# Ben-Bussch/Lunar_Module_Ascent_Trajectory_Optimiser

Hardware: AMD Instinct MI355X
Metric: solved ascent NLPs/sec (N=200 collocation nodes) (higher is better)
Workload: dtype f64; 1 GPU; BASELINE.json configs[2]: 4096-NLP Isp x dry-mass sweep (64x64, Isp 300-320 s, dry mass 2345-2545 kg), N=200 nodes, backward Euler (reference NODES=2), DCOST applied (the script's MV move penalty 1e-05, Launch_Optimiser.py:99, as an l1 term: the model the reference declares); move_penalty=True, batch_per_gpu=4096, global_batch=4096, n_nodes=200, parallelism=problem-sharded x1, gather only, converged=4096, of=4096

## Files before the change

include/ascent.h:

```cpp
#ifndef ASCENT_H
#define ASCENT_H
#include <stdint.h>

#ifdef __cplusplus
extern "C" {
#endif

typedef struct ascent_params {
  double G;
  double M;
  double R0;
  double Ft;
  double M0;
  double mdot;
  double fuel_mass;
  double mass_scalar;
  double ang_acc_max;
  double r_peri;
  double r_apo;
  double T_scale;
  double angle_ub;
  double tf_lb;
  double tf_ub;
  double dcost;
} ascent_params;

typedef struct ascent_opts {
  int32_t n_nodes;
  int32_t scheme;
  int32_t max_iter;
  int32_t warm_start;
  double tol;
  double mu_init;
  int32_t formulation;
  int32_t coarse_nodes;
  int32_t terminal;
  int32_t solver_path;
  int32_t move_penalty;
  int32_t reserved;
} ascent_opts;

enum ascent_status {
  ASCENT_OK = 0,
  ASCENT_E_ARG = -1,
  ASCENT_E_HIP = -2,
  ASCENT_E_NODEVICE = -3,
  ASCENT_E_NOMEM = -4,
  ASCENT_E_NOTERM = -5
};

enum ascent_problem_status {
  ASCENT_CONVERGED = 0,
  ASCENT_MAX_ITER = 1,
  ASCENT_LINESEARCH_FAILED = 2,
  ASCENT_REGULARISATION_FAILED = 3
};

#define ASCENT_BLOB_ROWS(n_nodes) (21 * ((n_nodes) - 1) + 10)
#define ASCENT_TRAJ_FIELDS 10

int ascent_version(void);
int ascent_device_count(void);
const char *ascent_strerror(int code);

int ascent_solve_batch(const ascent_params *p, int64_t batch, const ascent_opts *o,
                       const double *guess_or_null, double *traj_out, double *tf_out,
                       int32_t *status_out, int32_t *iters_out, double *sol_blob_out_or_null,
                       int device_id, void *hip_stream_or_null, int ptr_is_device);

int ascent_eval_nodes(const ascent_params *p, int64_t batch, const ascent_opts *o,
                      const double *iterate, double *defects, double *jac_blocks,
                      double *hess_blocks, int device_id);

int ascent_kkt_step(const ascent_params *p, int64_t batch, const ascent_opts *o,
                    const double *iterate, const double *mu, const double *delta_w, double *step,
                    int32_t *inertia_out, int device_id);

enum ascent_path { ASCENT_PATH_AUTO = 0, ASCENT_PATH_FUSED = 1, ASCENT_PATH_SPLIT_LANE = 2, ASCENT_PATH_SPLIT_WIDE = 3,
                   ASCENT_PATH_DENSE = 4,
                   ASCENT_PATH_PERSIST = 5  };
int ascent_default_path(int64_t batch, const ascent_opts *o);
int ascent_workspace_layout(int64_t batch, const ascent_opts *o, int64_t *out4);
int ascent_eval_nodes_path(const ascent_params *p, int64_t batch, const ascent_opts *o,
                           const double *iterate, double *defects, double *jac_blocks,
                           double *hess_blocks, int device_id, int path);
int ascent_kkt_step_path(const ascent_params *p, int64_t batch, const ascent_opts *o,
                         const double *iterate, const double *mu, const double *delta_w, double *step,
                         int32_t *inertia_out, int device_id, int path);

int ascent_dense_records(const ascent_params *p, int64_t batch, const ascent_opts *o, const double *iterate,
                         double *records, int device_id);

int ascent_coast_batch(const ascent_params *p, int64_t batch, const double *final_state, int32_t coast_nodes,
                       double *coast_traj, double *coast_tf, double *apsides, int device_id,
                       void *hip_stream_or_null, int ptr_is_device);

int ascent_param_sensitivity(const ascent_params *p, int64_t batch, const ascent_opts *o,
                             const double *sol_blob, double *grad_out,
                             int device_id, void *hip_stream_or_null, int ptr_is_device);

#define ASCENT_FLIGHT_ROWS 10
#define ASCENT_FLIGHT_MAX_SUBSTEPS 4096
int ascent_fly_batch(const ascent_params *p, int64_t batch, const ascent_opts *o, const double *sol_blob,
                     int32_t substeps, double *flown_traj_out_or_null, double *local_err_out_or_null,
                     double *summary_out, int device_id, void *hip_stream_or_null, int ptr_is_device);

int ascent_flight_jacobian(const ascent_params *p, int64_t batch, const ascent_opts *o, const double *sol_blob,
                           int32_t substeps, double *jac_out, double *jac_u_out_or_null, int device_id,
                           void *hip_stream_or_null, int ptr_is_device);

#define ASCENT_TRIM_ROWS 10
int ascent_trim_batch(const ascent_params *p, int64_t batch, const ascent_opts *o, const double *sol_blob, int32_t substeps,
                      int32_t rounds, double tol, double *trim_blob_out, double *summary_out, int device_id,
                      void *hip_stream_or_null, int ptr_is_device);

#define ASCENT_DISPERSE_COLS 24
#define ASCENT_DISPERSE_ROWS 9
#define ASCENT_DISPERSE_STAT_ROWS 82
#define ASCENT_DISPERSE_MAX_SAMPLES 65536
int ascent_disperse_batch(const ascent_params *p, int64_t batch, const ascent_opts *o, const double *sol_blob,
                          int32_t substeps, int32_t samples, const double *xi, const double *sigma,
                          const double *sigma_u_or_null, double *stats_out, double *samples_out_or_null, int device_id,
                          void *hip_stream_or_null, int ptr_is_device);

#define ASCENT_GUIDE_ROWS 5
int ascent_guidance_gains(const ascent_params *p, int64_t batch, const ascent_opts *o, const double *sol_blob, int32_t substeps,
                          const double *weights, double *gain_u_out, double *gain_t_out, double *summary_out,
                          double *jac_cl_out_or_null, double *jac_u_cl_out_or_null, int device_id, void *hip_stream_or_null,
                          int ptr_is_device);

#define ASCENT_GUIDED_SAMPLE_ROWS 12
int ascent_disperse_guided_batch(const ascent_params *p, int64_t batch, const ascent_opts *o, const double *sol_blob,
                                 int32_t substeps, int32_t samples, const double *xi, const double *sigma,
                                 const double *sigma_u_or_null, const double *gain_u, const double *gain_t_or_null,
                                 const double *stretch_max_or_null, double *stats_out, double *samples_out_or_null,
                                 int device_id, void *hip_stream_or_null, int ptr_is_device);

#define ASCENT_NAV_ROWS 8
#define ASCENT_GUIDE_FF_ROWS 7
int ascent_guidance_feedforward(const ascent_params *p, int64_t batch, const ascent_opts *o, const double *sol_blob,
                                int32_t substeps, const double *weights, const double *ff_dir, const double *ff_know_or_null,
                                double *gain_u_out, double *gain_t_out, double *ff_u_out, double *ff_t_out, double *summary_out,
                                double *jac_cl_out_or_null, double *jac_u_cl_out_or_null, double *jac_nav_out_or_null,
                                int device_id, void *hip_stream_or_null, int ptr_is_device);

int ascent_disperse_navigated_batch(const ascent_params *p, int64_t batch, const ascent_opts *o, const double *sol_blob,
                                    int32_t substeps, int32_t samples, const double *xi, const double *sigma,
                                    const double *sigma_u_or_null, const double *gain_u, const double *gain_t_or_null,
                                    const double *stretch_max_or_null, const double *ff_u_or_null, const double *ff_t_or_null,
                                    const double *ff_know_or_null, const double *xi_nav_or_null, const double *sigma_nav_or_null,
                                    double *stats_out, double *samples_out_or_null, int device_id, void *hip_stream_or_null,
                                    int ptr_is_device);

#define ASCENT_HISTORY_QUANTITIES 10
#define ASCENT_HISTORY_ROWS 52
int ascent_disperse_history_batch(const ascent_params *p, int64_t batch, const ascent_opts *o, const double *sol_blob,
                                  int32_t substeps, int32_t samples, const double *xi, const double *sigma,
                                  const double *sigma_u_or_null, const double *gain_u_or_null, const double *gain_t_or_null,
                                  const double *stretch_max_or_null, const double *ff_u_or_null, const double *ff_t_or_null,
                                  const double *ff_know_or_null, const double *xi_nav_or_null, const double *sigma_nav_or_null,
                                  int32_t node_stride, double *stats_out, double *samples_out_or_null, double *hist_out,
                                  double *hist_samples_out_or_null, int device_id, void *hip_stream_or_null, int ptr_is_device);

int ascent_kkt_solve(int64_t batch, int32_t n_nodes, int32_t bs, int32_t nb, const double *diag, const double *lower,
                     const double *upper, const double *border, const double *border_diag, const double *rhs,
                     double *sol, int device_id, int algo);

double ascent_last_kernel_ms(int device_id);

#ifdef __cplusplus
}
#endif
#endif
```

lunar_module_ascent_trajectory_optimiser_amd/_lib.py:

```python
from __future__ import annotations

import ctypes as C
import os

HERE = os.path.dirname(os.path.abspath(__file__))
LIB_PATH = os.path.join(HERE, "csrc", "libascent.so")

_dp = C.POINTER(C.c_double)
_ip = C.POINTER(C.c_int32)


class AscentParamsC(C.Structure):
    _fields_ = [(n, C.c_double) for n in (
        "G", "M", "R0", "Ft", "M0", "mdot", "fuel_mass", "mass_scalar", "ang_acc_max", "r_peri",
        "r_apo", "T_scale", "angle_ub", "tf_lb", "tf_ub", "dcost")]


class AscentOptsC(C.Structure):
    _fields_ = [("n_nodes", C.c_int32), ("scheme", C.c_int32), ("max_iter", C.c_int32),
                ("warm_start", C.c_int32), ("tol", C.c_double), ("mu_init", C.c_double),
                ("formulation", C.c_int32), ("coarse_nodes", C.c_int32), ("terminal", C.c_int32),
                ("solver_path", C.c_int32), ("move_penalty", C.c_int32), ("reserved", C.c_int32)]


SYMBOLS = ("ascent_version", "ascent_device_count", "ascent_strerror", "ascent_solve_batch",
           "ascent_eval_nodes", "ascent_kkt_step", "ascent_eval_nodes_path", "ascent_kkt_step_path",
           "ascent_dense_records", "ascent_coast_batch", "ascent_kkt_solve", "ascent_last_kernel_ms", "ascent_default_path",
           "ascent_workspace_layout", "ascent_param_sensitivity", "ascent_fly_batch", "ascent_flight_jacobian",
           "ascent_trim_batch", "ascent_disperse_batch", "ascent_guidance_gains", "ascent_disperse_guided_batch",
           "ascent_guidance_feedforward", "ascent_disperse_navigated_batch", "ascent_disperse_history_batch")
PATHS = {"auto": 0, "fused": 1, "split_lane": 2, "split_wide": 3, "dense": 4, "persist": 5}

_lib = None


class AscentLibraryError(RuntimeError):
    pass


def hip_runtimes_mapped() -> list[str]:
    seen = []
    try:
        with open("/proc/self/maps") as f:
            for line in f:
                path = line.rsplit(None, 1)[-1] if "/" in line else ""
                if "libamdhip64" in os.path.basename(path) and path not in seen:
                    seen.append(path)
    except OSError:
        pass
    return seen


def _bind_hip_runtime():
    if hip_runtimes_mapped() or os.environ.get("ASCENT_HIP_RUNTIME", "auto") == "system":
        return
    import importlib.util
    try:
        spec = importlib.util.find_spec("torch")
    except (ImportError, ValueError):
        spec = None
    if spec is None or not spec.origin:
        return
    cand = os.path.join(os.path.dirname(spec.origin), "lib", "libamdhip64.so")
    if os.path.exists(cand):
        try:
            C.CDLL(cand, mode=C.RTLD_GLOBAL)
        except OSError as e:
            import warnings
            warnings.warn(f"could not map {cand} ({e}); libascent.so binds to the system HIP runtime")


def require_single_hip_runtime():
    m = hip_runtimes_mapped()
    if len(m) > 1:
        raise AscentLibraryError(
            "two HIP runtimes are mapped into this process (" + ", ".join(m) + "): libascent.so was bound to one before torch "
            "loaded the other, so torch's device pointers and streams cannot be handed to it.  Import this package with "
            "ASCENT_HIP_RUNTIME unset (it then maps torch's runtime first), or `import torch` before the first solve.")


def load():
    global _lib
    if _lib is not None:
        return _lib
    if not os.path.exists(LIB_PATH):
        raise AscentLibraryError(
            f"{LIB_PATH} not found: build it with `python -m lunar_module_ascent_trajectory_optimiser_amd.build` "
            "(hipcc --offload-arch=gfx950).  There is no CPU fallback.")
    _bind_hip_runtime()
    L = C.CDLL(LIB_PATH)
    for s in SYMBOLS:
        if not hasattr(L, s):
            raise AscentLibraryError(f"{LIB_PATH} does not export {s}")
    L.ascent_version.restype = C.c_int
    L.ascent_device_count.restype = C.c_int
    L.ascent_strerror.restype = C.c_char_p
    L.ascent_strerror.argtypes = [C.c_int]
    L.ascent_last_kernel_ms.restype = C.c_double
    L.ascent_last_kernel_ms.argtypes = [C.c_int]
    L.ascent_solve_batch.restype = C.c_int
    L.ascent_solve_batch.argtypes = [C.c_void_p, C.c_int64, C.POINTER(AscentOptsC), C.c_void_p, C.c_void_p,
                                     C.c_void_p, C.c_void_p, C.c_void_p, C.c_void_p, C.c_int, C.c_void_p, C.c_int]
    L.ascent_eval_nodes.restype = C.c_int
    L.ascent_eval_nodes.argtypes = [C.c_void_p, C.c_int64, C.POINTER(AscentOptsC), C.c_void_p, C.c_void_p,
                                    C.c_void_p, C.c_void_p, C.c_int]
    L.ascent_kkt_step.restype = C.c_int
    L.ascent_kkt_step.argtypes = [C.c_void_p, C.c_int64, C.POINTER(AscentOptsC), C.c_void_p, C.c_void_p,
                                  C.c_void_p, C.c_void_p, C.c_void_p, C.c_int]
    L.ascent_eval_nodes_path.restype = C.c_int
    L.ascent_eval_nodes_path.argtypes = L.ascent_eval_nodes.argtypes + [C.c_int]
    L.ascent_kkt_step_path.restype = C.c_int
    L.ascent_kkt_step_path.argtypes = L.ascent_kkt_step.argtypes + [C.c_int]
    L.ascent_default_path.restype = C.c_int
    L.ascent_default_path.argtypes = [C.c_int64, C.POINTER(AscentOptsC)]
    L.ascent_workspace_layout.restype = C.c_int
    L.ascent_workspace_layout.argtypes = [C.c_int64, C.POINTER(AscentOptsC), C.POINTER(C.c_int64)]
    L.ascent_dense_records.restype = C.c_int
    L.ascent_dense_records.argtypes = [C.c_void_p, C.c_int64, C.POINTER(AscentOptsC), C.c_void_p, C.c_void_p, C.c_int]
    L.ascent_kkt_solve.restype = C.c_int
    L.ascent_kkt_solve.argtypes = [C.c_int64, C.c_int32, C.c_int32, C.c_int32] + [C.c_void_p] * 7 + [C.c_int, C.c_int]
    L.ascent_coast_batch.restype = C.c_int
    L.ascent_coast_batch.argtypes = [C.c_void_p, C.c_int64, C.c_void_p, C.c_int32, C.c_void_p, C.c_void_p, C.c_void_p,
                                     C.c_int, C.c_void_p, C.c_int]
    L.ascent_param_sensitivity.restype = C.c_int
    L.ascent_param_sensitivity.argtypes = [C.c_void_p, C.c_int64, C.POINTER(AscentOptsC), C.c_void_p, C.c_void_p, C.c_int,
                                           C.c_void_p, C.c_int]
    L.ascent_fly_batch.restype = C.c_int
    L.ascent_fly_batch.argtypes = [C.c_void_p, C.c_int64, C.POINTER(AscentOptsC), C.c_void_p, C.c_int32, C.c_void_p, C.c_void_p,
                                   C.c_void_p, C.c_int, C.c_void_p, C.c_int]
    L.ascent_flight_jacobian.restype = C.c_int
    L.ascent_flight_jacobian.argtypes = [C.c_void_p, C.c_int64, C.POINTER(AscentOptsC), C.c_void_p, C.c_int32, C.c_void_p, C.c_void_p,
                                         C.c_int, C.c_void_p, C.c_int]
    L.ascent_trim_batch.restype = C.c_int
    L.ascent_trim_batch.argtypes = [C.c_void_p, C.c_int64, C.POINTER(AscentOptsC), C.c_void_p, C.c_int32, C.c_int32, C.c_double,
                                    C.c_void_p, C.c_void_p, C.c_int, C.c_void_p, C.c_int]
    L.ascent_disperse_batch.restype = C.c_int
    L.ascent_disperse_batch.argtypes = [C.c_void_p, C.c_int64, C.POINTER(AscentOptsC), C.c_void_p, C.c_int32, C.c_int32, C.c_void_p,
                                        C.c_void_p, C.c_void_p, C.c_void_p, C.c_void_p, C.c_int, C.c_void_p, C.c_int]
    L.ascent_guidance_gains.restype = C.c_int
    L.ascent_guidance_gains.argtypes = [C.c_void_p, C.c_int64, C.POINTER(AscentOptsC), C.c_void_p, C.c_int32] + [C.c_void_p] * 6 + [
        C.c_int, C.c_void_p, C.c_int]
    L.ascent_disperse_guided_batch.restype = C.c_int
    L.ascent_disperse_guided_batch.argtypes = [C.c_void_p, C.c_int64, C.POINTER(AscentOptsC), C.c_void_p, C.c_int32, C.c_int32] + [
        C.c_void_p] * 8 + [C.c_int, C.c_void_p, C.c_int]
    L.ascent_guidance_feedforward.restype = C.c_int
    L.ascent_guidance_feedforward.argtypes = [C.c_void_p, C.c_int64, C.POINTER(AscentOptsC), C.c_void_p, C.c_int32] + [C.c_void_p] * 11 + [
        C.c_int, C.c_void_p, C.c_int]
    L.ascent_disperse_navigated_batch.restype = C.c_int
    L.ascent_disperse_navigated_batch.argtypes = [C.c_void_p, C.c_int64, C.POINTER(AscentOptsC), C.c_void_p, C.c_int32, C.c_int32] + [
        C.c_void_p] * 13 + [C.c_int, C.c_void_p, C.c_int]
    L.ascent_disperse_history_batch.restype = C.c_int
    L.ascent_disperse_history_batch.argtypes = [C.c_void_p, C.c_int64, C.POINTER(AscentOptsC), C.c_void_p, C.c_int32, C.c_int32] + [
        C.c_void_p] * 11 + [C.c_int32] + [C.c_void_p] * 4 + [C.c_int, C.c_void_p, C.c_int]
    _lib = L
    return L


def check(rc: int):
    if rc != 0:
        raise AscentLibraryError(f"libascent error {rc}: {load().ascent_strerror(rc).decode()}")
```

lunar_module_ascent_trajectory_optimiser_amd/csrc/ascent_dense.hip:

```cpp
#include <hip/hip_runtime.h>

#include <cstdio>
#include <cstdlib>

#include "ascent.h"
#include "ascent_device.hpp"
#include "ascent_tile.hpp"
#include "ascent_dense.hpp"
#include "ascent_blocktri.hpp"
#include "ascent_flight_dev.hpp"

using namespace ascent;

namespace {

constexpr int NIT = 26;
constexpr int O_Z = 0, O_U = 7, O_L = 8, O_ZB = 15;
constexpr int O_LU = 21, O_PP = 22, O_PN = 23, O_ZP = 24, O_ZN = 25;
constexpr int NV_GA = 0, NV_GB = 8, NV_P = 16, NNV = 27;
constexpr int G_JA = 0, G_JB = 1, G_HAA = 2, G_HAB = 3, G_HBB = 4, G_V = 5, NGRID = 6;
constexpr int F_EA = 0, F_LA = 1, F_EL2 = 2, F_GAIN = 3;
constexpr int FWD_DOUBLES = 3 * 64 + 16;
enum {
  X_STATE, X_ITERS, X_STATUS, X_CUR, X_FIRST, X_LS, X_MU, X_NUP, X_DWL, X_ALPHA, X_ADU, X_PHI0, X_DM, X_C1, X_SL,
// ... 8 lines not shown
struct DGeo {
  int K, scheme, terminal, dc;
  __host__ __device__ size_t nlp_doubles() const {
    return (size_t)K * (3 * NIT + NNV + NGRID * 64 + FWD_DOUBLES) + NSCAL;
  }
  __host__ __device__ size_t off_it(int buf) const { return (size_t)buf * NIT * K; }
  __host__ __device__ size_t off_st() const { return (size_t)2 * NIT * K; }
  __host__ __device__ size_t off_nv() const { return (size_t)3 * NIT * K; }
  __host__ __device__ size_t off_rec() const { return (size_t)(3 * NIT + NNV) * K; }
  __host__ __device__ size_t off_fwd() const { return off_rec() + (size_t)K * NGRID * 64; }
  __host__ __device__ size_t off_sc() const { return off_fwd() + (size_t)K * FWD_DOUBLES; }
};

ASC_DEV Scal load_scal(const double *sc, int r0) {
  Scal s;
  s.th = sc[r0 + S_TH]; s.zlt = sc[r0 + S_ZLT]; s.zut = sc[r0 + S_ZUT]; s.s1 = sc[r0 + S_S1]; s.s2 = sc[r0 + S_S2];
  s.zs1 = sc[r0 + S_ZS1]; s.zs2 = sc[r0 + S_ZS2]; s.nu3 = sc[r0 + S_NU3]; s.nu1 = sc[r0 + S_NU1]; s.nu2 = sc[r0 + S_NU2];
  return s;
}
ASC_DEV void store_scal(double *sc, int r0, const Scal &s) {
  sc[r0 + S_TH] = s.th; sc[r0 + S_ZLT] = s.zlt; sc[r0 + S_ZUT] = s.zut; sc[r0 + S_S1] = s.s1; sc[r0 + S_S2] = s.s2;
  sc[r0 + S_ZS1] = s.zs1; sc[r0 + S_ZS2] = s.zs2; sc[r0 + S_NU3] = s.nu3; sc[r0 + S_NU1] = s.nu1; sc[r0 + S_NU2] = s.nu2;
}
ASC_DEV Scal trial_scal(const Der &d, const Scal &s, const Scal &ds, double alpha, double adu, double mu, bool first) {
  Scal t = s;
  if (first) return t;
  t.th += alpha * ds.th; t.s1 += alpha * ds.s1; t.s2 += alpha * ds.s2;
  t.nu3 += alpha * ds.nu3; t.nu1 += alpha * ds.nu1; t.nu2 += alpha * ds.nu2;
  t.zlt = clipz(s.zlt + adu * ds.zlt, t.th - d.tlb, mu);
  t.zut = clipz(s.zut + adu * ds.zut, d.tub - t.th, mu);
  t.zs1 = clipz(s.zs1 + adu * ds.zs1, t.s1, mu);
  t.zs2 = clipz(s.zs2 + adu * ds.zs2, t.s2, mu);
  return t;
}

__global__ __launch_bounds__(WAVE) void d_init(const ascent_params *params, long batch, DGeo g, double *ws,
                                               const double *guess, int warm, double mu_init, int probe,
                                               const double *probe_mu) {
  const long p = blockIdx.y;
  const int k = blockIdx.x * WAVE + threadIdx.x, K = g.K;
  if (k >= K) return;
  double *w = ws + (size_t)p * g.nlp_doubles();
  const Der d = derive_t(params[p], g.terminal);
  const int asked_warm = warm;
  if (warm && !(guess[(21L * K + S_TH) * batch + p] > 0.0)) warm = 0;
  const double tf0 = 0.9, dr = 0.166, aend = 0.5, vp = sqrt(d.vp2), dt0 = (1.0 / K) * d.T * tf0;
  const double sdr = sin(dr), cdr = cos(dr);
  const double xf = -d.rhof * sdr, yf = d.rhof * cdr - d.rho0;
  double z[7], l[7], zb[6], u;
  if (warm) {
    ASC_UNROLL
    for (int i = 0; i < 7; i++) {
      z[i] = guess[(7L * k + i) * batch + p];
      l[i] = guess[(8L * K + 7L * k + i) * batch + p];
    }
    u = guess[(7L * K + k) * batch + p];
    ASC_UNROLL
    for (int b = 0; b < 6; b++) zb[b] = guess[(15L * K + 6L * k + b) * batch + p];
  } else {
    const double fr = (double)(k + 1) / K;
    z[IX] = fr * xf; z[IY] = fr * yf; z[IVX] = -fr * vp * cdr; z[IVY] = -fr * vp * sdr; z[IA] = fr * aend;
    z[IW] = aend / (K * dt0); z[IM] = d.mrate * dt0 * (k + 1);
    u = 0.0;
  }
  if (!probe) {
    z[IA] = push_in(z[IA], 0.0, d.aub);
    z[IM] = push_in(z[IM], 0.0, 1.0);
    u = push_in(u, -1.0, 1.0);
  }
  ASC_UNROLL
  for (int b = 0; b < 6; b++) zb[b] = warm == 2 ? (probe ? zb[b] : fmax(zb[b], 1e-12)) : 1.0;
  ASC_UNROLL
  for (int i = 0; i < 7; i++) l[i] = warm == 2 ? l[i] : 0.0;
  double *it = w + g.off_it(0), *st = w + g.off_st();
  ASC_UNROLL
  for (int i = 0; i < 7; i++) { it[(O_Z + i) * K + k] = z[i]; it[(O_L + i) * K + k] = l[i]; }
  it[O_U * K + k] = u;
  ASC_UNROLL
  for (int b = 0; b < 6; b++) it[(O_ZB + b) * K + k] = zb[b];
  for (int r = 0; r < NIT; r++) st[r * K + k] = 0.0;
  if (g.dc) {
    double up = (k > 0 && warm) ? guess[(7L * K + k - 1) * batch + p] : 0.0;
    if (k > 0 && !probe) up = push_in(up, -1.0, 1.0);
    const double dl = u - up, eps = warm ? 1e-4 : 1e-2, dc = params[p].dcost;
    it[O_LU * K + k] = 0.0;
    it[O_PP * K + k] = fmax(dl, 0.0) + eps; it[O_PN * K + k] = fmax(-dl, 0.0) + eps;
    it[O_ZP * K + k] = dc; it[O_ZN * K + k] = dc;
  }
  if (k != K - 1) return;
  double *sc = w + g.off_sc();
  Scal s;
  if (warm) {
    const double *gs = guess + (21L * K) * batch + p;
    s.th = gs[S_TH * batch]; s.zlt = gs[S_ZLT * batch]; s.zut = gs[S_ZUT * batch]; s.s1 = gs[S_S1 * batch];
    s.s2 = gs[S_S2 * batch]; s.zs1 = gs[S_ZS1 * batch]; s.zs2 = gs[S_ZS2 * batch]; s.nu3 = gs[S_NU3 * batch];
    s.nu1 = gs[S_NU1 * batch]; s.nu2 = gs[S_NU2 * batch];
  } else {
    s.th = tf0;
  }
  if (!probe) s.th = push_in(s.th, d.tlb, d.tub);
  const Terminal tm = terminal_of(d, z);
  if (probe) {
  } else if (warm != 2) {
    s.s1 = fmax(tm.g1, 1e-2); s.s2 = fmax(tm.g2, 1e-2);
    s.zlt = s.zut = s.zs1 = s.zs2 = 1.0;
    s.nu3 = s.nu1 = s.nu2 = 0.0;
  } else {
    s.s1 = fmax(s.s1, 1e-10); s.s2 = fmax(s.s2, 1e-10);
    s.zlt = fmax(s.zlt, 1e-12); s.zut = fmax(s.zut, 1e-12);
    s.zs1 = fmax(s.zs1, 1e-12); s.zs2 = fmax(s.zs2, 1e-12);
  }
  for (int r = 0; r < NSCAL; r++) sc[r] = 0.0;
  store_scal(sc, X_S, s);
  sc[X_STATE] = ST_TRIAL; sc[X_FIRST] = 1.0; sc[X_STATUS] = ASCENT_MAX_ITER;
  sc[X_MU] = probe ? probe_mu[p] : ((asked_warm && !warm) ? 0.1 : mu_init);
  sc[X_NUP] = 1.0;
}

struct QMap { int q; double c; };

ASC_DEV void h4_full(const double *H10, double H4[4][4]) {
  H4[0][0] = H10[0]; H4[0][1] = H4[1][0] = H10[1]; H4[0][2] = H4[2][0] = H10[2]; H4[0][3] = H4[3][0] = H10[3];
  H4[1][1] = H10[4]; H4[1][2] = H4[2][1] = H10[5]; H4[1][3] = H4[3][1] = H10[6];
  H4[2][2] = H10[7]; H4[2][3] = H4[3][2] = H10[8]; H4[3][3] = H10[9];
}

__global__ __launch_bounds__(WAVE) void d_eval(const ascent_params *params, long batch, DGeo g, double *ws) {
  const long p = blockIdx.y;
  const int k = blockIdx.x * WAVE + threadIdx.x, K = g.K;
  double *w = ws + (size_t)p * g.nlp_doubles();
  double *sc = w + g.off_sc();
  if ((int)sc[X_STATE] != ST_TRIAL || k >= K) return;
  const Der d = derive_t(params[p], g.terminal);
  const bool first = sc[X_FIRST] != 0.0;
  const double alpha = first ? 0.0 : sc[X_ALPHA], adu = first ? 0.0 : sc[X_ADU], mu = sc[X_MU];
  const Scal s = load_scal(sc, X_S), ds = load_scal(sc, X_D);
  const Scal stt = trial_scal(d, s, ds, alpha, adu, mu, first);
  const int cur = (int)sc[X_CUR];
  const double *ic = w + g.off_it(cur), *st = w + g.off_st();
  double *in = w + g.off_it(1 - cur), *nv = w + g.off_nv(), *rec = w + g.off_rec() + (size_t)k * NGRID * 64;
  const double hT = (1.0 / K) * d.T, dt = hT * stt.th;
  const double wa = g.scheme == 0 ? 0.0 : g.scheme == 1 ? 0.5 : 1.0 / 6.0;
  const double wm = g.scheme == 2 ? 4.0 / 6.0 : 0.0;
  const double wb = g.scheme == 0 ? 1.0 : g.scheme == 1 ? 0.5 : 1.0 / 6.0;
  const double sa = dt * wa, sm = dt * wm, sb = dt * wb, e8 = 0.125 * dt, h8 = 0.125 * hT;
  double za[7], zb[7], lam[7], zbd[6], u;
  ASC_UNROLL
  for (int i = 0; i < 7; i++) {
    zb[i] = ic[(O_Z + i) * K + k] + alpha * st[(O_Z + i) * K + k];
    za[i] = k ? ic[(O_Z + i) * K + k - 1] + alpha * st[(O_Z + i) * K + k - 1] : 0.0;
    lam[i] = ic[(O_L + i) * K + k] + alpha * st[(O_L + i) * K + k];
  }
  u = ic[O_U * K + k] + alpha * st[O_U * K + k];
  const double dist[6] = {zb[IA], d.aub - zb[IA], zb[IM], 1.0 - zb[IM], u + 1.0, 1.0 - u};
  const double mlo = mu * 1e-10, mhi = mu * 1e10;
  ASC_UNROLL
  for (int b = 0; b < 6; b++) {
    double v = ic[(O_ZB + b) * K + k];
    if (!first) { const double id = rcp(dist[b]); v = fmin(fmax(v + adu * st[(O_ZB + b) * K + k], mlo * id), mhi * id); }
    zbd[b] = v;
    in[(O_ZB + b) * K + k] = v;
  }
  ASC_UNROLL
  for (int i = 0; i < 7; i++) { in[(O_Z + i) * K + k] = zb[i]; in[(O_L + i) * K + k] = lam[i]; }
  in[O_U * K + k] = u;
  double lu = 0.0, pp = 1.0, pn = 1.0, zp = 0.0, zn = 0.0, cu = 0.0;
  if (g.dc) {
    const double up = k ? ic[O_U * K + k - 1] + alpha * st[O_U * K + k - 1] : 0.0;
    lu = ic[O_LU * K + k] + alpha * st[O_LU * K + k];
    pp = ic[O_PP * K + k] + alpha * st[O_PP * K + k];
    pn = ic[O_PN * K + k] + alpha * st[O_PN * K + k];
    zp = ic[O_ZP * K + k]; zn = ic[O_ZN * K + k];
    if (!first) {
      const double ip = rcp(pp), in_ = rcp(pn);
      zp = fmin(fmax(zp + adu * st[O_ZP * K + k], mlo * ip), mhi * ip);
      zn = fmin(fmax(zn + adu * st[O_ZN * K + k], mlo * in_), mhi * in_);
    }
    in[O_LU * K + k] = lu; in[O_PP * K + k] = pp; in[O_PN * K + k] = pn; in[O_ZP * K + k] = zp; in[O_ZN * K + k] = zn;
    cu = u - up - pp + pn;
  }
  if (k == K - 1) store_scal(sc, X_T, stt);
  double Ga[8], Gb[8], Gm[8], Hw[10], fa[7], fb[7], fm[7], zm[7], ax, ay;
  ASC_UNROLL
  for (int i = 0; i < 8; i++) { Ga[i] = 0.0; Gm[i] = 0.0; }
  ASC_UNROLL
  for (int i = 0; i < 7; i++) { fa[i] = 0.0; fm[i] = 0.0; zm[i] = 0.0; }
  accel<1>(d, zb[IX], zb[IY], zb[IA], zb[IM], 0.0, 0.0, ax, ay, Gb, nullptr);
  rhs_f(d, zb, u, ax, ay, fb);
  if (g.scheme != 0) {
    accel<1>(d, za[IX], za[IY], za[IA], za[IM], 0.0, 0.0, ax, ay, Ga, nullptr);
    rhs_f(d, za, u, ax, ay, fa);
  }
  double H4m[4][4];
  ASC_UNROLL
  for (int i = 0; i < 4; i++) {
    ASC_UNROLL
    for (int j = 0; j < 4; j++) H4m[i][j] = 0.0;
  }
  double gm[7], mth[7];
// ... 1170 lines not shown
```

lunar_module_ascent_trajectory_optimiser_amd/csrc/ascent_hs.hip:

```cpp
#include <hip/hip_runtime.h>

#pragma clang fp contract(on)

#include <cstdio>
#include <cstdlib>

#include "ascent.h"
#include "ascent_device.hpp"
#include "ascent_tile.hpp"
#include "ascent_persist.hpp"
#include "ascent_persist_dev.hpp"

using namespace ascent;

namespace {

typedef __attribute__((address_space(3))) double ldbl;
constexpr int HCH = 12, HCW = 48;
constexpr int LDH = 49;
constexpr int H_GA = 0, H_GM = 8, H_GB = 16, H_EB = 24, H_ES = 28, H_W = 32, H_R0 = 42, H_C = 45, H_JT = 52, H_H = 59, H_RZ = 69,
              H_GT = 76, H_ROWS = 83;
constexpr int C_PSI = 0, C_GA = 7, C_HA = 14, C_WA = 21, C_OM = 23, C_TG = 27, C_N = 34;


// ... 306 lines not shown
    ASC_UNROLL
    for (int i = 0; i < 10; i++) stage[(H_W + i) * LDH + col] = -sm * pt.Hm[i];
    ASC_UNROLL
    for (int i = 0; i < 7; i++) { stage[(H_C + i) * LDH + col] = cc[i]; stage[(H_JT + i) * LDH + col] = Jth[i]; }
  }
  double gan[7], han[7], wan[2];
  ASC_UNROLL
  for (int i = 0; i < 7; i++) { gan[i] = __shfl_down(q.ga[i], 1); han[i] = __shfl_down(Hath[i], 1); }
  wan[0] = __shfl_down(q.wa[0], 1); wan[1] = __shfl_down(q.wa[1], 1);
  if (on) {
    if (k == K - 1) {
      ASC_UNROLL
      for (int i = 0; i < 7; i++) { gan[i] = 0.0; han[i] = 0.0; }
      wan[0] = 0.0; wan[1] = 0.0;
    } else if (lastl) {
      ASC_UNROLL
      for (int i = 0; i < 7; i++) { gan[i] = carry[C_GA + i]; han[i] = carry[C_HA + i]; }
      wan[0] = carry[C_WA]; wan[1] = carry[C_WA + 1];
    }
    double Hn[10], Gx[8], t1, t2;
    accel<2>(d, z[IX], z[IY], z[IA], z[IM], q.wb[0] + wan[0], q.wb[1] + wan[1], t1, t2, Gx, Hn);
    const double dist[6] = {z[IA], d.aub - z[IA], z[IM], 1.0 - z[IM], u + 1.0, 1.0 - u};
    double id[6];
    ASC_UNROLL
    for (int b = 0; b < 6; b++) id[b] = rcp(dist[b]);
    ASC_UNROLL
    for (int i = 0; i < 10; i++) Hn[i] = -Hn[i];
    Hn[7] += zb6[0] * id[0] + zb6[1] * id[1];
    Hn[9] += zb6[2] * id[2] + zb6[3] * id[3];
    ASC_UNROLL
    for (int i = 0; i < 10; i++) stage[(H_H + i) * LDH + col] = Hn[i];
    ASC_UNROLL
    for (int i = 0; i < 7; i++) {
      double rz = q.gb[i] + gan[i];
      if (i == IA) rz += mu * (id[1] - id[0]);
      if (i == IM) rz += mu * (id[3] - id[2]);
      stage[(H_RZ + i) * LDH + col] = rz;
      stage[(H_GT + i) * LDH + col] = Hbth[i] + han[i];
    }
    stage[H_R0 * LDH + col] = zb6[4] * id[4] + zb6[5] * id[5] + dw;
    stage[(H_R0 + 1) * LDH + col] = -bu * lw + mu * (id[5] - id[4]);
    stage[(H_R0 + 2) * LDH + col] = -hT * d.alpha * lw;
  }
  wsync();
  if (on && firstl) {
    ASC_UNROLL
    for (int i = 0; i < 7; i++) { carry[C_GA + i] = q.ga[i]; carry[C_HA + i] = Hath[i]; }
    carry[C_WA] = q.wa[0]; carry[C_WA + 1] = q.wa[1];
  }
  wsync();
  return Hthth;
}

constexpr int F_OUT = 49, A_RHS = 42, A_C = 49, A_J = 56;
template <int WIDE>
ASC_PASS double hs_eval_forward(const ldbl *dp, const gdbl *it, const gdbl *gains, ldbl *stage, int K, int Kp, int kn, bool on, int nl, int col,
                                double h, double hT, double dth, double dnu3, double carry_m) {
  const Der d = der_load(dp);
  const double bu = h * d.alpha;
  double x0m = 0.0, du00 = 0.0, ka[7], rc[7];
  HsJ J;
  if (on) {
    double z[7], zp[7];
    ASC_UNROLL
    for (int i = 0; i < 7; i++) {
      z[i] = it[(O_Z + i) * Kp + kn];
      const double pv = it[(O_Z + i) * Kp + (kn > 0 ? kn - 1 : 0)];
      zp[i] = kn > 0 ? pv : 0.0;
    }
    const double u_ = it[O_U * Kp + kn];
    ASC_UNROLL
    for (int i = 0; i < 7; i++) ka[i] = gains[(size_t)i * Kp + kn];
    du00 = -(gains[(size_t)7 * Kp + kn] + gains[(size_t)8 * Kp + kn] * dth + gains[(size_t)9 * Kp + kn] * dnu3);
    HsPts pt;
    hs_points<0>(d, zp, z, u_, h, 0.0, 0.0, pt);
    double cc[7], Jth[7], eb[4], es[4];
    hs_defect(pt, zp, z, h, hT, cc, Jth);
    hs_blocks(pt.Gb, pt.Gm, h, eb, es);
    hs_coeffs(pt.Ga, pt.Gm, pt.Gb, eb, es, h, bu, J);
    ASC_UNROLL
    for (int i = 0; i < 7; i++) rc[i] = cc[i] + Jth[i] * dth;
    x0m = -rc[IM];
  }
  double incl = x0m;
  ASC_UNROLL
  for (int sft = 1; sft < (WIDE ? 64 : 16); sft *= 2) {
    const double t = __shfl_up(incl, sft, WIDE ? 64 : 16);
    if (nl >= sft) incl += t;
  }
  const double dzm_k = carry_m + incl, dzm_p = dzm_k - x0m;
  carry_m += WIDE ? __shfl(incl, HCW - 1) : bcast16<HCH - 1>(incl);
  if (on) {
    constexpr int NC = 6, FS = 7;
    const double du00p = du00 - ka[IM] * dzm_p;
    double X[4][7], Ab[4][7];
    hs_rows(J, X, Ab);
    auto emit = [&](int i, const double *xr_, const double *ar) {
      const double bw = bu * xr_[IW];
      double v = bw * du00p + ar[IM] * dzm_p;
      ASC_UNROLL
      for (int j = 0; j < 7; j++) v -= xr_[j] * rc[j];
      ASC_UNROLL
      for (int j = 0; j < 6; j++) stage[(FS * i + j) * LDH + col] = ar[j] - bw * ka[j];
      stage[(FS * i + NC) * LDH + col] = v;
    };
    emit(IX, X[0], Ab[0]); emit(IY, X[1], Ab[1]); emit(IVX, X[2], Ab[2]); emit(IVY, X[3], Ab[3]);
    {
      const double xa[7] = {0, 0, 0, 0, 1.0, 0.5 * h, 0}, aa[7] = {0, 0, 0, 0, 1.0, h, 0};
      emit(IA, xa, aa);
      const double xw[7] = {0, 0, 0, 0, 0, 1.0, 0}, aw[7] = {0, 0, 0, 0, 0, 1.0, 0};
      emit(IW, xw, aw);
    }
    ASC_UNROLL
    for (int j = 0; j < 6; j++) stage[(42 + j) * LDH + col] = -ka[j];
    stage[48 * LDH + col] = du00p;
    stage[(F_OUT + 6) * LDH + col] = dzm_k;
  }
  wsync();
  return carry_m;
}

template <int TERM>
ASC_PASS double hs_eval_adjoint(const ldbl *dp, const ldbl *sc, const gdbl *it, const gdbl *stp, ldbl *stage, ldbl *carry, int K, int Kp, int kn,
                                bool on, bool lastl, bool firstl, int col, double h, double hT, double mu, double dw, double dth, double dnu3) {
  const Der d = der_load(dp);
  const double bu = h * d.alpha, e8 = 0.125 * h;
  double ccl = 0.0, ccn[7], rhs[7] = {0, 0, 0, 0, 0, 0, 0};
  double om[4] = {0, 0, 0, 0}, Hath[7] = {0, 0, 0, 0, 0, 0, 0}, Hbth[7];
  HsJ J;
  HsPts pt;
  HsDual q;
  ASC_UNROLL
  for (int i = 0; i < 7; i++) q.ga[i] = 0.0;
  q.wa[0] = 0.0; q.wa[1] = 0.0;
  double z[7], dz[7], zb6[4];
  if (on) {
    double zp[7], l[7], dzp[7];
    ASC_UNROLL
    for (int i = 0; i < 7; i++) {
      const int km = kn > 0 ? kn - 1 : 0;
      z[i] = it[(O_Z + i) * Kp + kn]; l[i] = it[(O_L + i) * Kp + kn]; dz[i] = stp[(O_Z + i) * Kp + kn];
      const double pv = it[(O_Z + i) * Kp + km], dpv = stp[(O_Z + i) * Kp + km];
      zp[i] = kn > 0 ? pv : 0.0; dzp[i] = kn > 0 ? dpv : 0.0;
    }
    const double u = it[O_U * Kp + kn];
    ASC_UNROLL
    for (int b = 0; b < 4; b++) zb6[b] = it[(O_ZB + b) * Kp + kn];
    hs_points<1>(d, zp, z, u, h, l[IVX], l[IVY], pt);
    hs_dual(pt, l, h, q);
    double Jth[7], Hthth, eb[4], es[4];
    hs_defect(pt, zp, z, h, hT, ccn, Jth);
    hs_theta(pt, q, h, hT, Hath, Hbth, Hthth);
    hs_blocks(pt.Gb, pt.Gm, h, eb, es);
    hs_coeffs(pt.Ga, pt.Gm, pt.Gb, eb, es, h, bu, J);
    ASC_UNROLL
    for (int i = 0; i < 7; i++) ccl += ccn[i] * l[i];
    const double xi[4] = {0.5 * (dzp[IX] + dz[IX]) + e8 * (dzp[IVX] - dz[IVX]), 0.5 * (dzp[IY] + dz[IY]) + e8 * (dzp[IVY] - dz[IVY]),
                          0.5 * (dzp[IA] + dz[IA]) + e8 * (dzp[IW] - dz[IW]), 0.5 * (dzp[IM] + dz[IM])};
    const double sm = (4.0 / 6.0) * h;
    const double *H = pt.Hm;
    om[0] = -sm * (H[0] * xi[0] + H[1] * xi[1] + H[2] * xi[2] + H[3] * xi[3]);
    om[1] = -sm * (H[1] * xi[0] + H[4] * xi[1] + H[5] * xi[2] + H[6] * xi[3]);
    om[2] = -sm * (H[2] * xi[0] + H[5] * xi[1] + H[7] * xi[2] + H[8] * xi[3]);
    om[3] = -sm * (H[3] * xi[0] + H[6] * xi[1] + H[8] * xi[2] + H[9] * xi[3]);
  }
  double gan[7], han[7], wan[2], omn[4];
  ASC_UNROLL
  for (int i = 0; i < 7; i++) { gan[i] = __shfl_down(q.ga[i], 1); han[i] = __shfl_down(Hath[i], 1); }
  wan[0] = __shfl_down(q.wa[0], 1); wan[1] = __shfl_down(q.wa[1], 1);
  ASC_UNROLL
  for (int r = 0; r < 4; r++) omn[r] = __shfl_down(om[r], 1);
  if (on) {
// ... 693 lines not shown
```

lunar_module_ascent_trajectory_optimiser_amd/csrc/ascent_persist.hip:

```cpp
#include <hip/hip_runtime.h>

#pragma clang fp contract(on)

#include <cstdio>
#include <cstdlib>

#include "ascent.h"
#include "ascent_device.hpp"
#include "ascent_tile.hpp"
#include "ascent_persist.hpp"
#include "ascent_persist_dev.hpp"

using namespace ascent;

namespace {


ASC_DEV void start_move(double *w, int Kp, int k, double u, double up, bool warm, double dcw) {
  const double dl = u - up, eps = warm ? 1e-4 : 1e-2;
  w[(R_IT + O_LU) * Kp + k] = 0.0;
  w[(R_IT + O_PP) * Kp + k] = fmax(dl, 0.0) + eps;
  w[(R_IT + O_PN) * Kp + k] = fmax(-dl, 0.0) + eps;
  w[(R_IT + O_ZP) * Kp + k] = dcw;
  w[(R_IT + O_ZN) * Kp + k] = dcw;
}
struct MovePivot { double ip, in_, sgp, sgn, rp, rn, Rd, gdl; };
ASC_DEV MovePivot move_pivot(double pp, double pn, double zp, double zn, double lu, double dcw, double mu, double dw) {
  MovePivot m;
  m.ip = rcp(pp); m.in_ = rcp(pn);
  m.sgp = zp * m.ip + dw; m.sgn = zn * m.in_ + dw;
  m.rp = dcw - mu * m.ip - lu; m.rn = dcw - mu * m.in_ + lu;
  const double isp = rcp(m.sgp), isn = rcp(m.sgn);
  m.Rd = rcp(isp + isn);
  m.gdl = m.Rd * (m.rp * isp - m.rn * isn);
  return m;
}

ASC_DEV void start_node(const Der &d, int K, int kk, int warm, bool probe, int form, double *z, double *l, double *zb, double &u) {
  if (!warm) {
    const double tf0 = 0.9, dr = 0.166, aend = 0.5, vp = sqrt(d.vp2), dt0 = (1.0 / K) * d.T * tf0;
    const double sdr = sin(dr), cdr = cos(dr);
    const double xf = -d.rhof * sdr, yf = d.rhof * cdr - d.rho0;
    const double fr = (double)(kk + 1) / K;
    z[IX] = fr * xf; z[IY] = fr * yf; z[IVX] = -fr * vp * cdr; z[IVY] = -fr * vp * sdr; z[IA] = fr * aend;
    z[IW] = aend / (K * dt0); z[IM] = d.mrate * dt0 * (kk + 1);
    u = 0.0;
    if (form == 1) {
      z[IW] = 0.0;
      u = z[IA] / (0.5 * d.aub) - 1.0;
    }
  }
  if (!probe) {
    z[IA] = push_in(z[IA], 0.0, d.aub);
    z[IM] = push_in(z[IM], 0.0, 1.0);
    u = push_in(u, -1.0, 1.0);
  }
  ASC_UNROLL
  for (int b = 0; b < 6; b++) zb[b] = probe ? zb[b] : warm == 2 ? fmax(zb[b], 1e-12) : 1.0;
  ASC_UNROLL
  for (int i = 0; i < 7; i++) l[i] = warm == 2 ? l[i] : 0.0;
}
ASC_DEV void start_scal(const Der &d, int warm, bool probe, const double *zK, Scal &s) {
  if (!warm) s.th = 0.9;
  if (!probe) s.th = push_in(s.th, d.tlb, d.tub);
  const Terminal tm = terminal_of(d, zK);
  if (probe) {
  } else if (warm != 2) {
    s.s1 = fmax(tm.g1, 1e-2); s.s2 = fmax(tm.g2, 1e-2);
    s.zlt = s.zut = s.zs1 = s.zs2 = 1.0;
    s.nu3 = s.nu1 = s.nu2 = 0.0;
  } else {
    s.s1 = fmax(s.s1, 1e-10); s.s2 = fmax(s.s2, 1e-10);
    s.zlt = fmax(s.zlt, 1e-12); s.zut = fmax(s.zut, 1e-12);
    s.zs1 = fmax(s.zs1, 1e-12); s.zs2 = fmax(s.zs2, 1e-12);
  }
}
ASC_DEV void store_start(double *w, int Kp, int k, const double *z, const double *l, const double *zb, double u) {
  ASC_UNROLL
  for (int i = 0; i < 7; i++) { w[(R_IT + O_Z + i) * Kp + k] = z[i]; w[(R_IT + O_L + i) * Kp + k] = l[i]; }
  w[(R_IT + O_U) * Kp + k] = u;
  ASC_UNROLL
  for (int b = 0; b < 6; b++) w[(R_IT + O_ZB + b) * Kp + k] = zb[b];
}

__global__ __launch_bounds__(WAVE) void p_init(const ascent_params *params, long batch, PGeo g, double *ws, const double *guess,
                                               int warm, double mu_init, const double *probe_mu, const double *probe_dw, int probe_kind) {
  const long p = blockIdx.y;
  const int k = blockIdx.x * WAVE + threadIdx.x, K = g.K, Kp = g.Kp;
  if (k >= Kp) return;
  double *w = ws + (size_t)p * g.nlp_doubles();
  const Der d = derive_t(params[p], g.term);
  const int asked_warm = warm;
  if (warm && !(guess[(21L * K + S_TH) * batch + p] > 0.0)) warm = 0;
  const bool probe = probe_mu != nullptr;
  double z[7], l[7], zb[6], u = 0.0;
  const int kk = k < K ? k : K - 1;
  if (warm) {
    ASC_UNROLL
    for (int i = 0; i < 7; i++) { z[i] = guess[(7L * kk + i) * batch + p]; l[i] = guess[(8L * K + 7L * kk + i) * batch + p]; }
    u = guess[(7L * K + kk) * batch + p];
    ASC_UNROLL
    for (int b = 0; b < 6; b++) zb[b] = guess[(15L * K + 6L * kk + b) * batch + p];
  }
  start_node(d, K, kk, warm, probe, g.form, z, l, zb, u);
  store_start(w, Kp, k, z, l, zb, u);
  if (g.mp) {
    const double ha = 0.5 * d.aub, f0 = (double)kk / K * 0.5;
    double up = kk == 0 ? (g.form == 1 ? -1.0 : 0.0) : warm ? guess[(7L * K + kk - 1) * batch + p] : (g.form == 1 ? f0 / ha - 1.0 : 0.0);
    if (kk > 0 && !probe) up = push_in(up, -1.0, 1.0);
    start_move(w, Kp, k, u, up, warm != 0, g.form == 1 ? params[p].dcost * ha : params[p].dcost);
  }
  if (k != K - 1) return;
  double *sc = w + (size_t)g.nrows() * Kp;
  Scal s;
  if (warm) {
    const double *gs = guess + (21L * K) * batch + p;
    s.th = gs[S_TH * batch]; s.zlt = gs[S_ZLT * batch]; s.zut = gs[S_ZUT * batch]; s.s1 = gs[S_S1 * batch];
    s.s2 = gs[S_S2 * batch]; s.zs1 = gs[S_ZS1 * batch]; s.zs2 = gs[S_ZS2 * batch]; s.nu3 = gs[S_NU3 * batch];
    s.nu1 = gs[S_NU1 * batch]; s.nu2 = gs[S_NU2 * batch];
  }
  start_scal(d, warm, probe, z, s);
  for (int r = 0; r < NSCAL; r++) sc[r] = 0.0;
  put_scal(sc, X_S, s);
  sc[X_STATE] = ST_TRIAL; sc[X_FIRST] = 1.0; sc[X_STATUS] = ASCENT_MAX_ITER;
  sc[X_MU] = (asked_warm && !warm) ? 0.1 : mu_init; sc[X_NUP] = 1.0;
  if (probe) { sc[X_MU] = probe_mu[p]; sc[X_PDW] = probe_dw[p]; sc[X_PROBE] = (double)probe_kind; }
}

__global__ __launch_bounds__(WAVE) void p_transfer(const ascent_params *params, long batch, PGeo gc, const double *wsc, PGeo gf,
                                                   double *wsf, double mu) {
  const long p = blockIdx.y;
  const int k = blockIdx.x * WAVE + threadIdx.x, Kc = gc.K, Kf = gf.K, Kpc = gc.Kp, Kpf = gf.Kp;
  if (k >= Kpf) return;
  const double *wc = wsc + (size_t)p * gc.nlp_doubles(), *scc = wc + (size_t)gc.nrows() * Kpc;
  double *wf = wsf + (size_t)p * gf.nlp_doubles();
  const Der d = derive_t(params[p], gf.term);
  const int warm = (int)scc[X_STATUS] == ASCENT_CONVERGED ? 2 : 0;
  const double *ic = wc + (size_t)((int)scc[X_CUR] * gc.nit()) * Kpc;
  double z[7], l[7], zb[6], u = 0.0, up = 0.0;
  const int kk = k < Kf ? k : Kf - 1;
  if (warm && gf.mp && kk > 0) {
    const double x = (double)kk / (double)Kf * (double)Kc;
    int j = (int)x;
    if (j > Kc - 1) j = Kc - 1;
    const double wt = x - (double)j;
    const int ja = j ? j - 1 : 0;
    const double a = ic[O_U * Kpc + ja], b = ic[O_U * Kpc + j];
    up = push_in(fma(wt, b - a, a), -1.0, 1.0);
  }
  if (warm) {
    const double x = (double)(kk + 1) / (double)Kf * (double)Kc;
    int j = (int)x;
    if (j > Kc - 1) j = Kc - 1;
    const double wt = x - (double)j;
    const int ja = j ? j - 1 : 0;
    const double zsc = (double)Kc / (double)Kf;
    ASC_UNROLL
    for (int i = 0; i < 7; i++) {
      const double a = j ? ic[(O_Z + i) * Kpc + ja] : ((gf.form == 1 && i == IA) ? ic[(O_Z + i) * Kpc] : 0.0), b = ic[(O_Z + i) * Kpc + j];
      z[i] = fma(wt, b - a, a);
      const double la = ic[(O_L + i) * Kpc + ja], lb = ic[(O_L + i) * Kpc + j];
      l[i] = fma(wt, lb - la, la);
    }
    { const double a = ic[O_U * Kpc + ja], b = ic[O_U * Kpc + j]; u = fma(wt, b - a, a); }
    ASC_UNROLL
    for (int b6 = 0; b6 < 6; b6++) {
      const double a = ic[(O_ZB + b6) * Kpc + ja], b = ic[(O_ZB + b6) * Kpc + j];
      zb[b6] = fma(wt, b - a, a) * zsc;
    }
  }
  start_node(d, Kf, kk, warm, false, gf.form, z, l, zb, u);
  store_start(wf, Kpf, k, z, l, zb, u);
  if (gf.mp) {
    if (kk == 0) up = gf.form == 1 ? -1.0 : 0.0;
    else if (!warm && gf.form == 1) up = push_in((double)kk / Kf * 0.5 / (0.5 * d.aub) - 1.0, -1.0, 1.0);
    start_move(wf, Kpf, k, u, up, warm != 0, gf.form == 1 ? params[p].dcost * 0.5 * d.aub : params[p].dcost);
  }
  if (k != Kf - 1) return;
  double *sc = wf + (size_t)gf.nrows() * Kpf;
  Scal s;
  if (warm) s = lds_scal(scc, X_S);
  start_scal(d, warm, false, z, s);
  for (int r = 0; r < NSCAL; r++) sc[r] = 0.0;
  put_scal(sc, X_S, s);
  sc[X_STATE] = ST_TRIAL; sc[X_FIRST] = 1.0; sc[X_STATUS] = ASCENT_MAX_ITER;
  sc[X_MU] = warm ? mu : 0.1; sc[X_NUP] = 1.0;
  sc[X_ITB] = scc[X_ITB] + scc[X_ITERS];
}

constexpr int FIN_WAVES = 8, FIN_SUB = CH / FIN_WAVES;
__global__ __launch_bounds__(WAVE * FIN_WAVES) void p_finish(const ascent_params *params, long batch, PGeo g, const double *ws, double *traj,
                                                 double *tf_out, int *status_out, int *iters_out, double *blob) {
  const long p = (long)blockIdx.y * WAVE + threadIdx.x;
  if (p >= batch) return;
  const int c = blockIdx.x, K = g.K, Kp = g.Kp, nt = K + 1;
  const double *w = ws + (size_t)p * g.nlp_doubles();
  const double *sc = w + (size_t)g.nrows() * Kp;
  const Der d = derive_t(params[p], g.term);
  const double *it = w + (size_t)((int)sc[X_CUR] * g.nit()) * Kp;
  if (c == 0 && threadIdx.y == 0) {
    const Scal s = lds_scal(sc, X_S);
    tf_out[p] = s.th;
    status_out[p] = (int)sc[X_STATUS];
    iters_out[p] = (int)sc[X_ITERS] + (int)sc[X_ITB];
    if (blob) {
      double *bs = blob + (21L * K) * batch + p;
      bs[S_TH * batch] = s.th; bs[S_ZLT * batch] = s.zlt; bs[S_ZUT * batch] = s.zut; bs[S_S1 * batch] = s.s1;
      bs[S_S2 * batch] = s.s2; bs[S_ZS1 * batch] = s.zs1; bs[S_ZS2 * batch] = s.zs2; bs[S_NU3 * batch] = s.nu3;
      bs[S_NU1 * batch] = s.nu1; bs[S_NU2 * batch] = s.nu2;
    }
    if (traj) {
      double ax, ay;
      accel<0>(d, 0.0, 0.0, 0.0, 0.0, 0.0, 0.0, ax, ay, nullptr, nullptr);
      const double v[10] = {0.0, 0.0, 0.0, 0.0, ax, ay, 0.0, 0.0, 0.0, 0.0};
      ASC_UNROLL
      for (int f = 0; f < 10; f++) traj[((long)f * nt) * batch + p] = v[f];
    }
  }
  for (int k = c * CH + threadIdx.y * FIN_SUB; k < min(K, c * CH + (threadIdx.y + 1) * FIN_SUB); k++) {
    double z[7];
    ASC_UNROLL
    for (int q = 0; q < 7; q++) z[q] = it[(O_Z + q) * Kp + k];
    const double u = it[O_U * Kp + k];
    if (blob) {
      ASC_UNROLL
      for (int q = 0; q < 7; q++) {
        blob[(7L * k + q) * batch + p] = z[q];
        blob[(8L * K + 7L * k + q) * batch + p] = it[(O_L + q) * Kp + k];
      }
      blob[(7L * K + k) * batch + p] = u;
      ASC_UNROLL
      for (int b = 0; b < 6; b++) blob[(15L * K + 6L * k + b) * batch + p] = it[(O_ZB + b) * Kp + k];
    }
    if (traj) {
      double ax, ay;
      accel<0>(d, z[IX], z[IY], z[IA], z[IM], 0.0, 0.0, ax, ay, nullptr, nullptr);
      const double v[10] = {z[IX], z[IY], z[IVX], z[IVY], ax, ay, z[IA], z[IW], u, z[IM]};
      ASC_UNROLL
      for (int f = 0; f < 10; f++) traj[((long)f * nt + k + 1) * batch + p] = v[f];
    }
  }
}

__global__ __launch_bounds__(WAVE) void p_probe_out(long batch, PGeo g, const double *ws, double *step, int *inertia) {
  const long p = blockIdx.y;
  const int k = blockIdx.x * WAVE + threadIdx.x, K = g.K, Kp = g.Kp;
  if (k >= K) return;
  const double *w = ws + (size_t)p * g.nlp_doubles();
  const double *sc = w + (size_t)g.nrows() * Kp, *stp = w + (size_t)g.r_st() * Kp;
  const bool ok = (int)sc[X_STATE] == ST_TRIAL;
  if (k == 0) {
    inertia[p] = ok ? 0 : 1;
    for (int r = 0; r < 10; r++) step[(21L * K + r) * batch + p] = ok ? sc[X_D + r] : 0.0;
  }
  ASC_UNROLL
  for (int i = 0; i < 7; i++) {
    step[(7L * k + i) * batch + p] = ok ? stp[(O_Z + i) * Kp + k] : 0.0;
    step[(8L * K + 7L * k + i) * batch + p] = ok ? stp[(O_L + i) * Kp + k] : 0.0;
  }
  step[(7L * K + k) * batch + p] = ok ? stp[O_U * Kp + k] : 0.0;
  ASC_UNROLL
  for (int b = 0; b < 6; b++) step[(15L * K + 6L * k + b) * batch + p] = ok ? stp[(O_ZB + b) * Kp + k] : 0.0;
}

__global__ __launch_bounds__(WAVE) void p_probe_rows_out(const ascent_params *params, long batch, PGeo g, const double *ws, double *defects,
                                                         double *jac, double *hess) {
  const long p = blockIdx.y;
  const int k = blockIdx.x * WAVE + threadIdx.x, K = g.K, Kp = g.Kp;
  if (k >= K) return;
  const double *w = ws + (size_t)p * g.nlp_doubles();
  const double *sc = w + (size_t)g.nrows() * Kp, *rows = w + (size_t)g.r_st() * Kp;
  const double *it = w + (size_t)((int)sc[X_CUR] * g.nit()) * Kp;
  const Der d = derive_t(params[p], g.term);
  const double a_ = it[(O_Z + IA) * Kp + k], m_ = it[(O_Z + IM) * Kp + k];
  const double siga = it[(O_ZB + 0) * Kp + k] * rcp(a_) + it[(O_ZB + 1) * Kp + k] * rcp(d.aub - a_);
  const double sigm = it[(O_ZB + 2) * Kp + k] * rcp(m_) + it[(O_ZB + 3) * Kp + k] * rcp(1.0 - m_);
  ASC_UNROLL
  for (int i = 0; i < 8; i++) jac[(8L * k + i) * batch + p] = rows[i * Kp + k];
  ASC_UNROLL
  for (int i = 0; i < 10; i++) hess[(10L * k + i) * batch + p] = rows[(8 + i) * Kp + k] - (i == 7 ? siga : i == 9 ? sigm : 0.0);
  ASC_UNROLL
  for (int i = 0; i < 7; i++) defects[(7L * k + i) * batch + p] = rows[(18 + i) * Kp + k];
}


template <int FORM>
ASC_DEV void ainv_vrows(const double *G, const double *E, double dt, double *rvx, double *rvy) {
  double c1[7], c2[7];
  c1[IX] = dt * G[0]; c1[IY] = dt * G[1]; c1[IVX] = 1.0; c1[IVY] = 0.0; c1[IA] = dt * G[2]; c1[IW] = FORM == 1 ? 0.0 : dt * c1[IA]; c1[IM] = dt * G[3];
  c2[IX] = dt * G[4]; c2[IY] = dt * G[5]; c2[IVX] = 0.0; c2[IVY] = 1.0; c2[IA] = dt * G[6]; c2[IW] = FORM == 1 ? 0.0 : dt * c2[IA]; c2[IM] = dt * G[7];
  ASC_UNROLL
  for (int i = 0; i < 7; i++) { rvx[i] = E[0] * c1[i] + E[1] * c2[i]; rvy[i] = E[2] * c1[i] + E[3] * c2[i]; }
}


struct TrialKeep { double G[8], F[7], dza, dzm, zb4, zb5, zpp, zpn; };

template <int SCHEME, int FORM, int MP = 0, int TERM = 0>
ASC_DEV void trial_primal(const Der &d, int K, int Kp, int k, const NodeIn &n, const NodeIn &dn, const TrialCtx &t, bool live,
                          double *in, Part &P, TrialKeep &kp) {
  const double alpha = t.alpha;
  double z[7], zp[7], zb[6];
  ASC_UNROLL
  for (int i = 0; i < 7; i++) { z[i] = n.z[i] + alpha * dn.z[i]; zp[i] = n.zp[i] + alpha * dn.zp[i]; }
  const double u = n.u + alpha * dn.u;
  const double dist[6] = {z[IA], d.aub - z[IA], z[IM], 1.0 - z[IM], u + 1.0, 1.0 - u};
  ASC_UNROLL
  for (int b = 0; b < 6; b++) {
    const double id = rcp(dist[b]);
    zb[b] = t.first ? n.zb[b] : fmin(fmax(n.zb[b] + t.adu * dn.zb[b], t.mlo * id), t.mhi * id);
  }
  if (live) {
    ASC_UNROLL
    for (int i = 0; i < 7; i++) in[(O_Z + i) * Kp + k] = z[i];
    in[O_U * Kp + k] = u;
    ASC_UNROLL
    for (int b = 0; b < 6; b++) in[(O_ZB + b) * Kp + k] = zb[b];
  }
  kp.zpp = 0.0; kp.zpn = 0.0;
  if constexpr (MP) {
    const double up = n.up + alpha * dn.up, pp = n.pp + alpha * dn.pp, pn = n.pn + alpha * dn.pn;
    const double ip = rcp(pp), in_ = rcp(pn);
    const double zpp = t.first ? n.zpp : fmin(fmax(n.zpp + t.adu * dn.zpp, t.mlo * ip), t.mhi * ip);
    const double zpn = t.first ? n.zpn : fmin(fmax(n.zpn + t.adu * dn.zpn, t.mlo * in_), t.mhi * in_);
// ... 97 lines not shown
                        double *in, Part &P) {
  TrialKeep kp;
  trial_primal<SCHEME, FORM, MP, TERM>(d, K, Kp, k, n, dn, t, live, in, P, kp);
  double l[7], ln[7];
  ASC_UNROLL
  for (int i = 0; i < 7; i++) { l[i] = n.l[i] + t.alpha * dn.l[i]; ln[i] = n.ln[i] + t.alpha * dn.ln[i]; }
  const double lu = MP ? n.lu + t.alpha * dn.lu : 0.0, lun = MP ? n.lun + t.alpha * dn.lun : 0.0;
  trial_dual<SCHEME, FORM, MP, TERM>(d, K, Kp, k, kp, l, ln, lu, lun, t, live, in, P);
}


template <int SCHEME, int FORM, int MP = 0, int TERM = 0, int WIDE = 0>
__global__ __launch_bounds__(WAVE) void p_solve(const ascent_params *params, long batch, PGeo g, double *ws, int max_iter, double tol) {
  using L = Lay<MP>;
  constexpr int NS = L::NS, NIT = L::NIT, R_ST = L::R_ST, R_KA = L::R_KA, R_K0 = L::R_K0, NROWS = L::NROWS;
  constexpr int S_G = L::S_G, S_E = L::S_E, S_H = L::S_H, S_F = L::S_F, S_C = L::S_C, S_RZ = L::S_RZ, S_GT = L::S_GT, S_SC = L::S_SC;
  constexpr int RL = NS;
  static_assert(FORM == 0 || SCHEME == 0, "the v1 formulation is restated with backward Euler");
  __shared__ double stage[L::S_ROWS * LDW];
  __shared__ double outb[L::OUT_ROWS * LDW];
  __shared__ double lds_t[NPW][NS][NS];
  __shared__ double lds_d[NPW][3][8];
  __shared__ double lsc[NPW][NSCAL];
  __shared__ double lds_c[NPW][8];
  constexpr int CHN = WIDE ? 64 : CH;
  const int lane = threadIdx.x, grp = lane >> 4, role = lane & 15;
  const int nl = WIDE ? lane : role;
  const int cbase = WIDE ? 0 : grp * 16;
  const long p = WIDE ? (long)blockIdx.x : (long)blockIdx.x * NPW + grp;
  const bool live = p < batch;
  const long pc = live ? p : batch - 1;
  const int K = g.K, Kp = g.Kp, nch = g.nch;
  double *w = ws + (size_t)pc * g.nlp_doubles();
  double *gsc = w + (size_t)NROWS * Kp;
  double *sc = lsc[WIDE ? 0 : grp];
  const Der d = TERM == 2 ? derive_t(params[pc], 2) : derive(params[pc]);
  static_assert(TERM == 0 || (TERM == 2 && FORM == 0), "terminal 2 is carried for the current formulation");
  for (int r = role; r < NSCAL; r += 16) sc[r] = gsc[r];
  if (role < 8) lds_d[grp][2][role] = 0.0;
  wsync();
  if (!live && role == 0) sc[X_STATE] = ST_DONE;
  wsync();
  const int col = grp * 16 + role;
  const double hT = (1.0 / K) * d.T;
  constexpr int IB = FORM == 1 ? IA : IW;
  const double dcw = MP ? (FORM == 1 ? params[pc].dcost * 0.5 * d.aub : params[pc].dcost) : 0.0;
  constexpr double UINIT = FORM == 1 ? -1.0 : 0.0;

  PROF_DECL
  for (int round = 0; round < 64 * (max_iter + 2); round++) {
    PROF(9);
    int state = (int)sc[X_STATE];
    if (__all(state == ST_DONE)) break;
    int pass = 0;
    do {
      if (state == ST_TRIAL) {
        const bool first = sc[X_FIRST] != 0.0;
        const double alpha = first ? 0.0 : sc[X_ALPHA], adu = first ? 0.0 : sc[X_ADU], mu = sc[X_MU];
        const Scal s = lds_scal(sc, X_S), ds = lds_scal(sc, X_D);
        const Scal stt = trial_scal(d, s, ds, alpha, adu, mu, first);
        const int cur = (int)sc[X_CUR];
        const double *ic = w + (size_t)(cur * NIT) * Kp, *stp = w + (size_t)R_ST * Kp;
        double *in = w + (size_t)((1 - cur) * NIT) * Kp;
        const double dt = hT * stt.th, be = dt * d.alpha;
        const double mlo = mu * 1e-10, mhi = mu * 1e10;
        Part P;
        if (sc[X_TEVAL] != 0.0) {
          P.rd = sc[X_P + 0]; P.cinf = sc[X_P + 1]; P.pmin = sc[X_P + 2]; P.pmax = sc[X_P + 3]; P.l1 = sc[X_P + 4];
          P.zsum = sc[X_P + 5]; P.rth = sc[X_P + 6]; P.c1 = sc[X_P + 7]; P.sl = sc[X_P + 8]; P.mv = sc[X_P + 9];
        } else {
          TrialCtx t;
          t.alpha = alpha; t.adu = adu; t.mlo = mlo; t.mhi = mhi; t.dt = dt; t.be = be; t.hT = hT; t.first = first; t.stt = stt; t.dcw = dcw;
          P.clear();
          for (int c = 0; c < nch; c++) {
            const int k = c * CHN + nl;
            if (k < K) {
              NodeIn n, dn;
              load_node<MP>(ic, Kp, K, k, n, UINIT);
              if (first) dn = NodeIn{};
              else load_node<MP>(stp, Kp, K, k, dn);
              trial_node<SCHEME, FORM, MP, TERM>(d, K, Kp, k, n, dn, t, live, in, P);
            }
          }
          P.template reduceW<MP, WIDE>();
        }
        double rd = P.rd, cinf = P.cinf, pmin = P.pmin, pmax = P.pmax, l1 = P.l1, zsum = P.zsum;
        const double rth = 1.0 + P.rth, c1 = P.c1, sl = P.sl;
        double nu_pen = sc[X_NUP], iters = sc[X_ITERS], mu2 = mu;
        int nstate = ST_FACTOR;
        bool accepted = true;
        if (!first) {
          const double phi0 = sc[X_PHI0], Dm = sc[X_DM];
          const double phit = (MP ? stt.th + dcw * P.mv : stt.th) - mu * sl + nu_pen * c1;
          if (!(isfinite(phit) && phit <= phi0 + 1e-8 * alpha * Dm + 2.220446049250313e-15 * fabs(phi0))) {
            accepted = false;
            const int ls = (int)sc[X_LS] + 1;
            wsync();
            if (role == 0) {
              sc[X_LS] = ls; sc[X_TEVAL] = 0.0;
              if (ls >= 40) { sc[X_STATUS] = ASCENT_LINESEARCH_FAILED; sc[X_STATE] = ST_DONE; }
              else sc[X_ALPHA] = 0.5 * alpha;
            }
          } else {
            iters += 1.0;
          }
        }
        if (accepted) {
          ErrParts e;
          e.rd = fmax(rd, fabs(rth - stt.zlt + stt.zut));
          e.rd = fmax(e.rd, fmax(fabs(-stt.nu1 - stt.zs1), fabs(-stt.nu2 - stt.zs2)));
          e.cinf = cinf;
          const double pr[4] = {(stt.th - d.tlb) * stt.zlt, (d.tub - stt.th) * stt.zut, stt.s1 * stt.zs1, stt.s2 * stt.zs2};
          ASC_UNROLL
          for (int q = 0; q < 4; q++) { pmin = fmin(pmin, pr[q]); pmax = fmax(pmax, pr[q]); }
          e.pmin = pmin; e.pmax = pmax;
          l1 += fabs(stt.nu3) + fabs(stt.nu1) + fabs(stt.nu2);
          zsum += stt.zlt + stt.zut + stt.zs1 + stt.zs2;
          e.sd = fmax(100.0, (l1 + zsum) / (double)((MP ? 16 : 13) * K + 7)) * 0.01;
          int status = -1;
          const bool probe = sc[X_PROBE] != 0.0;
          if (probe) { }
          else if (e.err(0.0) <= tol) { status = ASCENT_CONVERGED; nstate = ST_DONE; }
          else if ((int)iters >= max_iter) { status = ASCENT_MAX_ITER; nstate = ST_DONE; }
          else {
            while (mu2 > tol * 0.1 && e.err(mu2) <= 10.0 * mu2) {
              mu2 = fmax(tol * 0.1, fmin(0.2 * mu2, mu2 * sqrt(mu2)));
              nu_pen = 1.0;
            }
          }
#ifdef PERSIST_TRACE
          if (role == 0 && p == PERSIST_TRACE && K > 100)
            printf("[persist] K=%d iter %2d mu %.1e E0 %.2e (dual %.1e primal %.1e compl %.1e..%.1e s_d %.2g) alpha %.3g adu %.3g ls %d dw %.1e nu_pen %.2g c1 %.2e\n", K, (int)iters, mu,
                   e.err(0.0), e.rd, e.cinf, e.pmin, e.pmax, e.sd, alpha, adu, (int)sc[X_LS], sc[X_DWL], nu_pen, c1);
          if (role == 0 && p == PERSIST_TRACE && K > 100)
            printf("[persist]      dual rows: nodes %.2e | th %.2e s1 %.2e s2 %.2e\n", rd, fabs(rth - stt.zlt + stt.zut), fabs(-stt.nu1 - stt.zs1), fabs(-stt.nu2 - stt.zs2));
#endif
          wsync();
          if (role == 0) {
            put_scal(sc, X_S, stt);
            sc[X_CUR] = 1 - cur; sc[X_FIRST] = 0.0; sc[X_ITERS] = iters; sc[X_LS] = 0.0; sc[X_C1] = c1; sc[X_SL] = sl; sc[X_RTH] = rth;
            sc[X_MU] = mu2; sc[X_NUP] = nu_pen; sc[X_DW] = probe ? sc[X_PDW] : 0.0; sc[X_STATE] = nstate; sc[X_TEVAL] = 0.0;
            if (MP) sc[X_MV] = P.mv;
            if (status >= 0) sc[X_STATUS] = status;
          }
        }
      }
      wsync();
      state = (int)sc[X_STATE];
    } while (__builtin_expect(__any(state == ST_TRIAL) && ++pass < 41, 0));
    PROF(0);
    state = (int)sc[X_STATE];
    if (__any(state == ST_FACTOR)) {
      const bool act = state == ST_FACTOR;
      const Scal s = lds_scal(sc, X_S);
      const double mu = sc[X_MU], dw = sc[X_DW];
      const double *it = w + (size_t)((int)sc[X_CUR] * NIT) * Kp;
      const double dt = hT * s.th, be = dt * d.alpha, ith = rcp(s.th), cs = SCHEME == 1 ? 0.5 * dt : dt;
      const double ha = 0.5 * d.aub, bu = FORM == 1 ? ha : be;
      const double hTc = SCHEME == 1 ? 0.5 * hT : hT;
      int grow[NS];
      double gsgn[NS];
      {
        constexpr int hmap[8] = {0, 1, -1, -1, 2, -1, 3, -1};
        constexpr int hrow[4][4] = {{0, 1, 2, 3}, {1, 4, 5, 6}, {2, 5, 7, 8}, {3, 6, 8, 9}};
        ASC_UNROLL
        for (int i = 0; i < NS; i++) {
          int row = S_H; double sgn = 0.0;
// ... 178 lines not shown
              for (int i = 0; i < NS; i++) a[i] += role == i ? dw : 0.0;
            }
            double b[NS];
            solveAT<FORM>(G, E, cs, a, b);
            if constexpr (MP) b[7] = a[7] + bu * b[IB];
            if (colr) {
              ASC_UNROLL
              for (int i = 0; i < NS; i++) lds_t[grp][role][i] = b[i];
              wsync();
              double t[NS];
              ASC_UNROLL
              for (int l2 = 0; l2 < NS; l2++) t[l2] = lds_t[grp][l2][role];
              solveAT<FORM>(G, E, cs, t, b);
              if constexpr (MP) b[7] = t[7] + bu * b[IB];
            }
            double mw[NS], D, coef;
            if constexpr (MP) {
              ASC_UNROLL
              for (int i = 0; i < NS; i++) mw[i] = bcast16<7>(b[i]);
              D = R0 + mw[7];
            } else {
              ASC_UNROLL
              for (int i = 0; i < NS; i++) mw[i] = bu * bcast16<IB>(b[i]);
              D = R0 + dw + bu * mw[IB];
            }
            const double iD = rcp(D);
            if constexpr (MP) {
              const double rsel = role == RL ? ru0 : 0.0;
              coef = (b[7] - rsel) * iD;
            } else {
              const double ru = ru0 + mu * bur, gu = FORM == 1 ? 0.0 : ru0 * ith;
              const double rsel = role == 7 ? ru : role == 8 ? gu : 0.0;
              coef = (bu * b[IB] - rsel) * iD;
            }
            ASC_UNROLL
            for (int i = 0; i < NS; i++) a[i] = b[i] - mw[i] * coef;
            outb[rowK + cj] = role < NS + 3 ? coef : D;
            if (colr) {
              double d0 = 0.0, d1 = 0.0;
              ASC_UNROLL
              for (int i = 0; i < NS; i++) {
                d0 -= a[i] * cc[i];
                if (i < 7) d1 += a[i] * rc1[i];
              }
              lds_d[grp][0][role] = d0;
              lds_d[grp][1][role] = d1;
            }
            wsync();
            {
              double prc[NS];
              ASC_UNROLL
              for (int i = 0; i < NS; i++) prc[i] = lds_d[grp][drow][i];
              double uu = 0.0, vv = 0.0;
              ASC_UNROLL
              for (int i = 0; i < NS; i++) {
                const double pj = a[i] - prc[i], sj = a[i] + pj;
                if (i < 7) uu += rc1[i] * sj;
                vv += cc[i] * sj;
                a[i] = pj;
              }
              U += uu; V += vv;
            }
          }
        }
        wsync();
        PROF(2);
        {
          const int k = c * CHN + nl;
          if (k < K && act) {
            if (live) {
              ASC_UNROLL
              for (int i = 0; i < NS + 3; i++) w[(size_t)(R_KA + i) * Kp + k] = outb[i * LDW + col];
            }
            const double k00 = outb[NS * LDW + col], k01 = outb[(NS + 1) * LDW + col], k02 = outb[(NS + 2) * LDW + col], D = outb[(NS + 3) * LDW + col];
            const double Dk1 = D * k01, Dk2 = D * k02;
            k10 += Dk1 * k00; k11 += Dk1 * k01; k12 += Dk1 * k02; k20 += Dk2 * k00; k22 += Dk2 * k02;
            if (!(D > 0.0)) bad = 1;
          }
        }
        wsync();
        PROF(3);
      }
      const double U0 = bcast16<RL>(U), U1 = bcast16<RL + 1>(U), V1 = bcast16<RL + 1>(V), U2 = bcast16<RL + 2>(U), V2 = bcast16<RL + 2>(V);
      k10 = gsumW<WIDE>(k10); k11 = gsumW<WIDE>(k11); k12 = gsumW<WIDE>(k12); k20 = gsumW<WIDE>(k20); k22 = gsumW<WIDE>(k22);
      bad = (int)gmaxW<WIDE>((double)bad);
      if (probe_rows) {
        if (act && role == 0) sc[X_STATE] = ST_DONE;
      } else if (act) {
        const double S10 = k10 + 0.5 * (U0 - V1), S11 = k11 + U1, S12 = k12 + 0.5 * U2, S20 = k20 - 0.5 * V2, S22 = k22;
        int ok = !bad;
        double dth = 0.0, dnu3 = 0.0;
        if (ok) {
          const double itl = rcp(s.th - d.tlb), itu = rcp(d.tub - s.th);
          const double rthp = sc[X_RTH] + mu * (itu - itl);
          const double sth = s.zlt * itl + s.zut * itu + dw;
          const double a11 = sth - S11, a12 = -S12, a22 = TERM == 2 ? -1.0 : -S22;
          const double b1 = -rthp + S10, b2 = -tm.e3 + S20;
          const double det = a11 * a22 - a12 * a12;
          if (det < 0.0) {
            const double idet = 1.0 / det;
            dth = (b1 * a22 - a12 * b2) * idet;
            dnu3 = (a11 * b2 - a12 * b1) * idet;
          } else {
            ok = 0;
          }
        }
        if (role == 0) {
          if (ok) {
            sc[X_DTH] = dth; sc[X_DNU3] = dnu3; sc[X_SIG1] = sig1; sc[X_SIG2] = sig2; sc[X_RS1] = rs1; sc[X_RS2] = rs2;
            sc[X_CG1] = tm.g1 - s.s1; sc[X_CG2] = tm.g2 - s.s2;
            sc[X_DWL] = dw; sc[X_STATE] = ST_FACTORED;
          } else {
            const double ndw = next_delta_w(dw, sc[X_DWL]);
            if (sc[X_PROBE] != 0.0) sc[X_STATE] = ST_DONE;
            else if (ndw > 1e10) { sc[X_STATUS] = ASCENT_REGULARISATION_FAILED; sc[X_STATE] = ST_DONE; }
            else sc[X_DW] = ndw;
          }
        }
      }
    }
    wsync();
    state = (int)sc[X_STATE];
    if (__any(state == ST_FACTORED)) {
      const bool act = state == ST_FACTORED;
      const Scal s = lds_scal(sc, X_S);
      const double mu = sc[X_MU], dw = sc[X_DWL], dth = sc[X_DTH], dnu3 = sc[X_DNU3];
      const double sig1 = sc[X_SIG1], sig2 = sc[X_SIG2], rs1 = sc[X_RS1], rs2 = sc[X_RS2];
      const double *it = w + (size_t)((int)sc[X_CUR] * NIT) * Kp;
      double *stp = w + (size_t)R_ST * Kp;
      const double dt = hT * s.th, be = dt * d.alpha, cs = SCHEME == 1 ? 0.5 * dt : dt, hTc = SCHEME == 1 ? 0.5 * hT : hT;
      const double ha = 0.5 * d.aub, bu = FORM == 1 ? ha : be;
      const double tau = fmax(0.99, 1.0 - mu);
      {
        constexpr int NC = 6 + MP, FS = NC + 1;
        const int fbase = (role < 7 ? FS * role : 0) * LDW;
        const int fout = (role < 6 ? role : role == 6 ? 7 : 8) * LDW;
        double yown = 0.0, carry_m = 0.0, carry_u = 0.0;
        double rmax = 0.0, gsum = 0.0, adu = 1.0, gmove = 0.0, clu = 0.0;
        double dzK[7] = {0, 0, 0, 0, 0, 0, 0};
        for (int c = 0; c < nch; c++) {
          const int kn = c * CHN + nl;
          const bool on = kn < K && act;
          double a_ = 0.5, m_ = 0.5, u_ = 0.0, zb[6] = {1, 1, 1, 1, 1, 1};
          double G[8], Gp[8], E[4], x0[7], ka[NS], du00 = 0.0;
          double x0u = 0.0, pp_ = 1.0, pn_ = 1.0, zpp_ = 0.0, zpn_ = 0.0, lu_ = 0.0;
          ASC_UNROLL
          for (int i = 0; i < 7; i++) x0[i] = 0.0;
          ASC_UNROLL
          for (int i = 0; i < NS; i++) ka[i] = 0.0;
          if (on) {
            double z[7], zp[7], F[7], ax, ay;
            ASC_UNROLL
            for (int i = 0; i < 7; i++) { z[i] = it[(O_Z + i) * Kp + kn]; zp[i] = kn > 0 ? it[(O_Z + i) * Kp + kn - 1] : 0.0; }
            u_ = it[O_U * Kp + kn];
            a_ = z[IA]; m_ = z[IM];
            ASC_UNROLL
            for (int b = 0; b < 6; b++) zb[b] = it[(O_ZB + b) * Kp + kn];
            ASC_UNROLL
            for (int i = 0; i < NS; i++) ka[i] = w[(size_t)(R_KA + i) * Kp + kn];
            if constexpr (MP) {
              pp_ = it[O_PP * Kp + kn]; pn_ = it[O_PN * Kp + kn]; zpp_ = it[O_ZP * Kp + kn]; zpn_ = it[O_ZN * Kp + kn]; lu_ = it[O_LU * Kp + kn];
              x0u = -(u_ - (kn > 0 ? it[O_U * Kp + kn - 1] : UINIT) - pp_ + pn_);
            }
            du00 = w[(size_t)R_K0 * Kp + kn] + w[(size_t)(R_K0 + 1) * Kp + kn] * dth + w[(size_t)(R_K0 + 2) * Kp + kn] * dnu3;
            accel<1>(d, z[IX], z[IY], z[IA], z[IM], 0.0, 0.0, ax, ay, G, nullptr);
            rhs_f<FORM>(d, z, u_, ax, ay, F);
            if (SCHEME == 1) {
              double Fb[7], axp, ayp;
              accel<1>(d, zp[IX], zp[IY], zp[IA], zp[IM], 0.0, 0.0, axp, ayp, Gp, nullptr);
              rhs_f<FORM>(d, zp, u_, axp, ayp, Fb);
              ASC_UNROLL
              for (int i = 0; i < 7; i++) F[i] = 0.5 * (F[i] + Fb[i]);
            }
            implicit_block(G, cs, E);
            ASC_UNROLL
            for (int i = 0; i < 7; i++) {
              x0[i] = hT * F[i] * dth - ((FORM == 1 && i == IA) ? z[IA] - ha * (u_ + 1.0) : z[i] - zp[i] - dt * F[i]);
              du00 -= ka[i] * x0[i];
            }
            if constexpr (MP) du00 -= ka[7] * x0u;
          }
          double incl = x0[IM];
          ASC_UNROLL
          for (int sft = 1; sft < CHN; sft *= 2) {
            const double t = __shfl_up(incl, sft, CHN);
            if (nl >= sft) incl += t;
          }
          const double dzm_k = carry_m + incl, dzm_p = dzm_k - x0[IM];
          carry_m += WIDE ? __shfl(incl, 63) : bcast16<15>(incl);
          if (on) {
            const double du00p = du00 - ka[IM] * dzm_p;
            double rvx[7], rvy[7];
            ainv_vrows<FORM>(G, E, cs, rvx, rvy);
            auto emit = [&](int i, const double *r, double aw) {
              const double bw = bu * aw;
              if constexpr (MP) stage[(FS * i + 6) * LDW + col] = bw * (1.0 - ka[7]);
              if (SCHEME == 1) {
                double m7[7], t[7];
                ASC_UNROLL
                for (int j = 0; j < 7; j++) m7[j] = r[j] - bw * ka[j];
                fzt_lambda(Gp, m7, t);
                ASC_UNROLL
                for (int j = 0; j < 7; j++) m7[j] += cs * t[j];
                double v = bw * (MP ? x0u + du00 : du00) + m7[IM] * dzm_p;
                ASC_UNROLL
                for (int j = 0; j < 7; j++) v += r[j] * x0[j];
                ASC_UNROLL
                for (int j = 0; j < 6; j++) stage[(FS * i + j) * LDW + col] = m7[j];
                stage[(FS * i + NC) * LDW + col] = v;
                return;
              }
              double v = bw * (MP ? x0u + du00p : du00p) + r[IM] * dzm_p;
              ASC_UNROLL
              for (int j = 0; j < 7; j++) v += r[j] * x0[j];
              ASC_UNROLL
              for (int j = 0; j < 6; j++) stage[(FS * i + j) * LDW + col] = (FORM == 1 && j == IA) ? 0.0 : r[j] - bw * ka[j];
              stage[(FS * i + NC) * LDW + col] = v;
            };
            emit(IVX, rvx, rvx[IB]);
            emit(IVY, rvy, rvy[IB]);
            {
              double r[7];
              ASC_UNROLL
              for (int j = 0; j < 7; j++) r[j] = (j == IX ? 1.0 : 0.0) + cs * rvx[j];
              emit(IX, r, cs * rvx[IB]);
              ASC_UNROLL
              for (int j = 0; j < 7; j++) r[j] = (j == IY ? 1.0 : 0.0) + cs * rvy[j];
              emit(IY, r, cs * rvy[IB]);
              ASC_UNROLL
              for (int j = 0; j < 7; j++) r[j] = j == IA ? 1.0 : (j == IW && FORM == 0) ? cs : 0.0;
              emit(IA, r, FORM == 1 ? 1.0 : cs);
              ASC_UNROLL
              for (int j = 0; j < 7; j++) r[j] = j == IW ? 1.0 : 0.0;
              emit(IW, r, FORM == 1 ? 0.0 : 1.0);
            }
            if constexpr (MP) {
              double kj[7], v0;
              if (SCHEME == 1) {
                double t[7];
                fzt_lambda(Gp, ka, t);
                ASC_UNROLL
                for (int j = 0; j < 7; j++) kj[j] = ka[j] + cs * t[j];
                v0 = du00 - kj[IM] * dzm_p;
              } else {
                ASC_UNROLL
                for (int j = 0; j < 7; j++) kj[j] = ka[j];
                v0 = du00p;
              }
              ASC_UNROLL
              for (int j = 0; j < 6; j++) stage[(FS * 6 + j) * LDW + col] = (FORM == 1 && j == IA) ? 0.0 : -kj[j];
              stage[(FS * 6 + 6) * LDW + col] = 1.0 - ka[7];
              stage[(FS * 6 + NC) * LDW + col] = x0u + v0;
            } else if (SCHEME == 1) {
              double t[7];
              fzt_lambda(Gp, ka, t);
              ASC_UNROLL
              for (int j = 0; j < 6; j++) stage[(42 + j) * LDW + col] = -(ka[j] + cs * t[j]);
              stage[48 * LDW + col] = du00 - (ka[IM] + cs * t[IM]) * dzm_p;
            } else {
              ASC_UNROLL
              for (int j = 0; j < 6; j++) stage[(42 + j) * LDW + col] = (FORM == 1 && j == IA) ? 0.0 : -ka[j];
              stage[48 * LDW + col] = du00p;
            }
            outb[6 * LDW + col] = dzm_k;
          }
          wsync();
          PROF(4);
          if (act) {
            const int jn = min(CHN, K - c * CHN);
            for (int jj = 0; jj < jn; jj++) {
              const int cj = cbase + jj;
              const double *sj = stage + fbase + cj;
              const double m0 = sj[0], m1 = sj[LDW], m2 = sj[2 * LDW], m3 = sj[3 * LDW], m4 = sj[4 * LDW], m5 = sj[5 * LDW], vv = sj[NC * LDW];
              const double b0 = bcast16<0>(yown), b1 = bcast16<1>(yown), b2 = bcast16<2>(yown), b3 = bcast16<3>(yown),
                           b4 = bcast16<4>(yown), b5 = bcast16<5>(yown);
              const double e0 = (vv + m0 * b0) + m2 * b2, e1 = m1 * b1 + m3 * b3, e2 = m4 * b4 + m5 * b5;
              if constexpr (MP) {
                const double m6 = sj[6 * LDW], b6 = bcast16<6>(yown);
                yown = ((e0 + e1) + e2) + m6 * b6;
              } else {
                yown = (e0 + e1) + e2;
              }
              outb[fout + cj] = yown;
            }
          }
          wsync();
          PROF(5);
          if (kn < K && act) {
            double dzn[8];
            ASC_UNROLL
            for (int i = 0; i < 8; i++) dzn[i] = outb[i * LDW + col];
            const double id[6] = {rcp(a_), rcp(d.aub - a_), rcp(m_), rcp(1.0 - m_), rcp(u_ + 1.0), rcp(1.0 - u_)};
            const double dza = dzn[IA], dzm = dzn[IM], du = dzn[7];
            if (kn == K - 1) cpy<7>(dzK, dzn);
            ASC_FTBR(rmax, id[0], dza); ASC_FTBR(rmax, id[1], -dza);
            ASC_FTBR(rmax, id[2], dzm); ASC_FTBR(rmax, id[3], -dzm);
            ASC_FTBR(rmax, id[4], du); ASC_FTBR(rmax, id[5], -du);
            gsum += dza * (id[1] - id[0]) + dzm * (id[3] - id[2]) + du * (id[5] - id[4]);
            const double dx3[3] = {dza, dzm, du};
            double dzb[6];
            ASC_UNROLL
            for (int b = 0; b < 3; b++) {
              const double zl = zb[2 * b], zu = zb[2 * b + 1];
              dzb[2 * b] = id[2 * b] * (mu - zl * dx3[b]) - zl;
              dzb[2 * b + 1] = id[2 * b + 1] * (mu + zu * dx3[b]) - zu;
              ASC_FTB(adu, zl, dzb[2 * b]);
              ASC_FTB(adu, zu, dzb[2 * b + 1]);
            }
            if (live) {
              ASC_UNROLL
              for (int i = 0; i < 7; i++) stp[(O_Z + i) * Kp + kn] = dzn[i];
              stp[O_U * Kp + kn] = du;
              ASC_UNROLL
              for (int b = 0; b < 6; b++) stp[(O_ZB + b) * Kp + kn] = dzb[b];
            }
            if constexpr (MP) {
              const double du_p = nl > 0 ? outb[7 * LDW + col - 1] : carry_u;
              const double ddel = (du - du_p) - x0u;
              const MovePivot mvp = move_pivot(pp_, pn_, zpp_, zpn_, lu_, dcw, mu, dw);
              const double dlu = mvp.Rd * ddel + mvp.gdl;
              double dpp, dpn;
              if (mvp.sgp >= mvp.sgn) { dpp = (dlu - mvp.rp) * rcp(mvp.sgp); dpn = dpp - ddel; }
              else { dpn = (-dlu - mvp.rn) * rcp(mvp.sgn); dpp = ddel + dpn; }
              const double dzp = mvp.ip * (mu - zpp_ * dpp) - zpp_, dzn_ = mvp.in_ * (mu - zpn_ * dpn) - zpn_;
              ASC_FTBR(rmax, mvp.ip, dpp); ASC_FTBR(rmax, mvp.in_, dpn);
              ASC_FTB(adu, zpp_, dzp); ASC_FTB(adu, zpn_, dzn_);
              gsum -= dpp * mvp.ip + dpn * mvp.in_;
              gmove += dpp + dpn;
              clu -= x0u * (lu_ + dlu);
              if (live) {
                stp[O_LU * Kp + kn] = dlu; stp[O_PP * Kp + kn] = dpp; stp[O_PN * Kp + kn] = dpn; stp[O_ZP * Kp + kn] = dzp; stp[O_ZN * Kp + kn] = dzn_;
              }
            }
          }
          if constexpr (MP) carry_u = outb[7 * LDW + cbase + CHN - 1];
          wsync();
          PROF(6);
        }
        rmax = gmaxW<WIDE>(rmax); gsum = gsumW<WIDE>(gsum); adu = gminW<WIDE>(adu);
        if constexpr (MP) { gmove = gsumW<WIDE>(gmove); clu = gsumW<WIDE>(clu); }
        ASC_UNROLL
        for (int i = 0; i < 7; i++) dzK[i] = gsumW<WIDE>(dzK[i]);
        double zK[7];
        ASC_UNROLL
        for (int i = 0; i < 7; i++) zK[i] = it[(O_Z + i) * Kp + K - 1];
        const Terminal tmK = TERM == 2 ? terminal_eval_any(d, zK) : terminal_eval(d, zK);
        Scal ds;
        ds.th = dth; ds.nu3 = dnu3;
        ds.s1 = sc[X_CG1] + tmK.g1g[0] * dzK[IX] + tmK.g1g[1] * dzK[IY];
        ds.s2 = sc[X_CG2] + tmK.g2g[0] * dzK[IVX] + tmK.g2g[1] * dzK[IVY];
        if constexpr (TERM == 2) {
          ds.s1 += tmK.g1v[0] * dzK[IVX] + tmK.g1v[1] * dzK[IVY];
          ds.s2 += tmK.g2p[0] * dzK[IX] + tmK.g2p[1] * dzK[IY];
        }
        ds.nu1 = sig1 * ds.s1 + rs1;
        ds.nu2 = sig2 * ds.s2 + rs2;
        ds.zs1 = mu / s.s1 - s.zs1 - s.zs1 / s.s1 * ds.s1;
        ds.zs2 = mu / s.s2 - s.zs2 - s.zs2 / s.s2 * ds.s2;
        const double dl_ = s.th - d.tlb, dU = d.tub - s.th;
        ds.zlt = mu / dl_ - s.zlt - s.zlt / dl_ * ds.th;
        ds.zut = mu / dU - s.zut + s.zut / dU * ds.th;
        double apr = 1.0;
        if (rmax * apr > tau) apr = tau / rmax;
        ASC_FTB(apr, dl_, ds.th); ASC_FTB(apr, dU, -ds.th);
        ASC_FTB(apr, s.s1, ds.s1); ASC_FTB(apr, s.s2, ds.s2);
        ASC_FTB(adu, s.zlt, ds.zlt); ASC_FTB(adu, s.zut, ds.zut);
        ASC_FTB(adu, s.zs1, ds.zs1); ASC_FTB(adu, s.zs2, ds.zs2);
        TrialCtx tc;
        tc.alpha = apr; tc.adu = adu; tc.mlo = mu * 1e-10; tc.mhi = mu * 1e10; tc.hT = hT; tc.first = false; tc.dcw = dcw;
        tc.stt = trial_scal(d, s, ds, apr, adu, mu, false);
        tc.dt = hT * tc.stt.th; tc.be = tc.dt * d.alpha;
        double *in = w + (size_t)((1 - (int)sc[X_CUR]) * NIT) * Kp;
        Part P;
        P.clear();
        const int abase = (role < 7 ? 6 * role : 0) * LDW;
        const int aout = (role < 7 ? role : 8) * LDW;
        const double aself = (role == IW || role == IM) ? 1.0 : 0.0;
        double lown = 0.0;
        double cl = 0.0, ccl = 0.0;
        for (int c = nch - 1; c >= 0; c--) {
          const int kn = c * CHN + nl;
          double ccn[7] = {0, 0, 0, 0, 0, 0, 0};
          TrialKeep kp;
          if (kn < K && act) {
            NodeIn n, dn;
            load_node<MP>(it, Kp, K, kn, n, UINIT);
            ASC_UNROLL
            for (int i = 0; i < 7; i++) { dn.z[i] = stp[(O_Z + i) * Kp + kn]; dn.zp[i] = kn > 0 ? stp[(O_Z + i) * Kp + kn - 1] : 0.0; }
            dn.u = stp[O_U * Kp + kn];
            ASC_UNROLL
            for (int b = 0; b < 6; b++) dn.zb[b] = stp[(O_ZB + b) * Kp + kn];
            if constexpr (MP) {
              dn.up = kn > 0 ? stp[O_U * Kp + kn - 1] : 0.0;
              dn.lu = stp[O_LU * Kp + kn];
              dn.lun = kn + 1 < K ? stp[O_LU * Kp + kn + 1] : 0.0;
              dn.pp = stp[O_PP * Kp + kn]; dn.pn = stp[O_PN * Kp + kn]; dn.zpp = stp[O_ZP * Kp + kn]; dn.zpn = stp[O_ZN * Kp + kn];
            }
            const double *dz = dn.z;
            double G[8], E[4], H[10], F[7], fl[7], lt[7], ax, ay;
            ASC_UNROLL
            for (int i = 0; i < 7; i++) lt[i] = SCHEME == 1 ? n.l[i] + n.ln[i] : n.l[i];
            accel<2>(d, n.z[IX], n.z[IY], n.z[IA], n.z[IM], -cs * lt[IVX], -cs * lt[IVY], ax, ay, G, H);
            rhs_f<FORM>(d, n.z, n.u, ax, ay, F);
            if (SCHEME == 1) {
              double Fb[7], axp, ayp;
              accel<0>(d, n.zp[IX], n.zp[IY], n.zp[IA], n.zp[IM], 0.0, 0.0, axp, ayp, nullptr, nullptr);
              rhs_f<FORM>(d, n.zp, n.u, axp, ayp, Fb);
              ASC_UNROLL
              for (int i = 0; i < 7; i++) F[i] = 0.5 * (F[i] + Fb[i]);
            }
            implicit_block(G, cs, E);
            fzt_lambda<FORM>(G, lt, fl);
            const double id0 = rcp(n.z[IA]), id1 = rcp(d.aub - n.z[IA]), id2 = rcp(n.z[IM]), id3 = rcp(1.0 - n.z[IM]);
            H[7] += n.zb[0] * id0 + n.zb[1] * id1;
            H[9] += n.zb[2] * id2 + n.zb[3] * id3;
            double r[7];
            ASC_UNROLL
            for (int i = 0; i < 7; i++) {
              const double rz = (FORM == 1 && i == IA) ? n.l[i] - cs * fl[i] : n.l[i] - cs * fl[i] - n.ln[i], gt = -hTc * fl[i];
              r[i] = -rz - gt * dth - dw * dz[i];
              ccn[i] = (FORM == 1 && i == IA) ? n.z[IA] - ha * (n.u + 1.0) : n.z[i] - n.zp[i] - dt * F[i];
              ccl += ccn[i] * n.l[i];
            }
            r[IA] -= mu * (id1 - id0);
            r[IM] -= mu * (id3 - id2);
// ... 20 lines not shown
              r[IX] -= s.nu3 * tm.e3g[0] + w1 * tm.g1g[0] + tm.e3g[0] * dnu3;
              r[IY] -= s.nu3 * tm.e3g[1] + w1 * tm.g1g[1] + tm.e3g[1] * dnu3;
              r[IVX] -= s.nu3 * tm.e3g[2] + w2 * tm.g2g[0] + tm.e3g[2] * dnu3;
              r[IVY] -= s.nu3 * tm.e3g[3] + w2 * tm.g2g[1] + tm.e3g[3] * dnu3;
              }
            }
            double wv[7];
            solveAT<FORM>(G, E, cs, r, wv);
            {
              double rvx[7], rvy[7];
              ainv_vrows<FORM>(G, E, cs, rvx, rvy);
              ASC_UNROLL
              for (int i = 0; i < 7; i++) {
                double nr[7];
                nr[IVX] = rvx[i]; nr[IVY] = rvy[i];
                nr[IX] = (i == IX ? 1.0 : 0.0) + cs * rvx[i];
                nr[IY] = (i == IY ? 1.0 : 0.0) + cs * rvy[i];
                nr[IA] = FORM == 1 ? 0.0 : i == IA ? 1.0 : i == IW ? cs : 0.0;
                nr[IW] = i == IW ? 1.0 : 0.0;
                nr[IM] = i == IM ? 1.0 : 0.0;
                if (SCHEME == 1) {
                  double t[7];
                  fz_mul(G, nr, t);
                  ASC_UNROLL
                  for (int j = 0; j < 7; j++) nr[j] += cs * t[j];
                }
                ASC_UNROLL
                for (int j = 0; j < 5; j++) stage[(6 * i + j) * LDW + col] = nr[j];
              }
            }
            ASC_UNROLL
            for (int i = 0; i < 7; i++) stage[(6 * i + 5) * LDW + col] = wv[i];
            trial_primal<SCHEME, FORM, MP, TERM>(d, K, Kp, kn, n, dn, tc, live, in, P, kp);
          }
          wsync();
          PROF(7);
          if (act) {
            const int jj0 = min(CHN, K - c * CHN) - 1;
            for (int jj = jj0; jj >= 0; jj--) {
              const int cj = cbase + jj;
              const double *sj = stage + abase + cj;
              const double n0 = sj[0], n1 = sj[LDW], n2 = sj[2 * LDW], n3 = sj[3 * LDW], n4 = sj[4 * LDW], wv = sj[5 * LDW];
              const double b0 = bcast16<0>(lown), b1 = bcast16<1>(lown), b2 = bcast16<2>(lown), b3 = bcast16<3>(lown), b4 = bcast16<4>(lown);
              const double e0 = (wv + aself * lown) + n0 * b0, e1 = n1 * b1 + n2 * b2, e2 = n3 * b3 + n4 * b4;
              lown = (e0 + e1) + e2;
              outb[aout + cj] = lown;
            }
          }
          wsync();
          double dl[7], dln[7];
          if (kn < K && act) {
            ASC_UNROLL
            for (int i = 0; i < 7; i++) {
              dl[i] = outb[i * LDW + col];
              dln[i] = kn + 1 < K ? (nl < CHN - 1 ? outb[i * LDW + col + 1] : lds_c[WIDE ? 0 : grp][i]) : 0.0;
              ccl += ccn[i] * dl[i];
            }
            if (live) {
              ASC_UNROLL
              for (int i = 0; i < 7; i++) stp[(O_L + i) * Kp + kn] = dl[i];
            }
          }
          wsync();
          PROF(8);
          if (kn < K && act) {
            if (nl == 0) {
              ASC_UNROLL
              for (int i = 0; i < 7; i++) lds_c[WIDE ? 0 : grp][i] = dl[i];
            }
            double l[7], ln[7], lu = 0.0, lun = 0.0;
            ASC_UNROLL
            for (int i = 0; i < 7; i++) {
              l[i] = it[(O_L + i) * Kp + kn] + tc.alpha * dl[i];
              ln[i] = (kn + 1 < K ? it[(O_L + i) * Kp + kn + 1] : 0.0) + tc.alpha * dln[i];
            }
            if constexpr (MP) {
              lu = it[O_LU * Kp + kn] + tc.alpha * stp[O_LU * Kp + kn];
              lun = (kn + 1 < K ? it[O_LU * Kp + kn + 1] : 0.0) + tc.alpha * (kn + 1 < K ? stp[O_LU * Kp + kn + 1] : 0.0);
            }
            trial_dual<SCHEME, FORM, MP, TERM>(d, K, Kp, kn, kp, l, ln, lu, lun, tc, live, in, P);
          }
          PROF(0);
        }
        P.template reduceW<MP, WIDE>();
        ccl = gsumW<WIDE>(ccl);
        if (act) {
          cl += ccl;
          const Terminal &tm = tmK;
          double gd = MP ? mu * gsum + dcw * gmove : mu * gsum;
          if constexpr (MP) cl += clu;
          gd += ds.th * (1.0 - mu / dl_ + mu / dU) - mu * ds.s1 / s.s1 - mu * ds.s2 / s.s2;
          cl += tm.e3 * (s.nu3 + ds.nu3) + sc[X_CG1] * (s.nu1 + ds.nu1) + sc[X_CG2] * (s.nu2 + ds.nu2);
          const double c1 = sc[X_C1], slog = sc[X_SL];
          double nu_pen = sc[X_NUP];
          const double curv = -gd + cl;
          if (c1 > 0.0) {
            const double need = (gd + 0.5 * fmax(curv, 0.0)) / (0.9 * c1);
            if (nu_pen < need) nu_pen = need + 1.0;
          }
          wsync();
          if (role == 0) {
            put_scal(sc, X_D, ds);
            sc[X_NUP] = nu_pen;
            sc[X_DM] = gd - nu_pen * c1;
            sc[X_PHI0] = (MP ? s.th + dcw * sc[X_MV] : s.th) - mu * slog + nu_pen * c1;
            sc[X_ALPHA] = apr; sc[X_ADU] = adu; sc[X_LS] = 0.0;
            sc[X_P + 0] = P.rd; sc[X_P + 1] = P.cinf; sc[X_P + 2] = P.pmin; sc[X_P + 3] = P.pmax; sc[X_P + 4] = P.l1;
            sc[X_P + 5] = P.zsum; sc[X_P + 6] = P.rth; sc[X_P + 7] = P.c1; sc[X_P + 8] = P.sl; sc[X_P + 9] = P.mv;
            sc[X_TEVAL] = 1.0;
            sc[X_STATE] = ST_TRIAL;
          }
        }
      }
    }
    wsync();
    if (sc[X_PROBE] != 0.0) break;
  }
  wsync();
  PROF_END;
  if (live)
    for (int r = role; r < NSCAL; r += 16) gsc[r] = sc[r];
}

}

namespace ascent {

static PGeo geo_of(int K, int form = 0, int mp = 0, int term = 0, int wide = 0, int scheme = 0) {
  PGeo g;
  const int ch = scheme == 2 ? hs_chunk_nodes(wide) : wide ? 64 : CH;
  g.K = K; g.nch = (K + ch - 1) / ch; g.Kp = (g.nch * ch + 15) / 16 * 16;
  g.form = form; g.mp = mp ? 1 : 0; g.term = term == 2 ? 2 : 0; g.wide = wide ? 1 : 0;
  return g;
}

static size_t level_doubles(int K, int mp) {
  size_t m = 0;
  for (int scheme = 0; scheme <= 2; scheme += 2)
    for (int wide = 0; wide <= 1; wide++) {
      const size_t n = geo_of(K, 0, mp, 0, wide, scheme).nlp_doubles();
      m = n > m ? n : m;
    }
  return m;
}
size_t persist_ws_bytes(int K, long batch, int mp) {
  const size_t b = (size_t)batch * level_doubles(K, mp) * sizeof(double) + 64;
  return (b + 255) & ~(size_t)255;
}
size_t persist_region1_offset(const int *levels, long batch, int mp) { return persist_ws_bytes(levels[0] - 1, batch, mp); }
size_t persist_level_bytes_used(int K, long batch, int mp) { return (size_t)batch * level_doubles(K, mp) * sizeof(double); }
size_t persist_ws_bytes_nested(const int *levels, int nlev, long batch, int mp) {
  size_t b = persist_region1_offset(levels, batch, mp);
  if (nlev > 1) b += persist_ws_bytes(levels[1] - 1, batch, mp);
  return b;
}

using SolveKernel = void (*)(const ascent_params *, long, PGeo, double *, int, double);
struct SolveVariant { int scheme, form, mp, term, wide; SolveKernel kernel; };
#define ASC_VARIANT(S, F, M, T, W) {S, F, M, T, W, p_solve<S, F, M, T, W>}
static const SolveVariant solve_variants[] = {
    ASC_VARIANT(1, 0, 1, 2, 1), ASC_VARIANT(0, 0, 1, 2, 1), ASC_VARIANT(1, 0, 0, 2, 1), ASC_VARIANT(0, 0, 0, 2, 1),
    ASC_VARIANT(1, 0, 1, 0, 1), ASC_VARIANT(0, 1, 1, 0, 1), ASC_VARIANT(0, 1, 0, 0, 1), ASC_VARIANT(0, 0, 1, 0, 1),
    ASC_VARIANT(1, 0, 0, 0, 1), ASC_VARIANT(0, 0, 0, 0, 1),
    ASC_VARIANT(1, 0, 1, 2, 0), ASC_VARIANT(0, 0, 1, 2, 0), ASC_VARIANT(1, 0, 0, 2, 0), ASC_VARIANT(0, 0, 0, 2, 0),
    ASC_VARIANT(1, 0, 1, 0, 0), ASC_VARIANT(0, 1, 1, 0, 0), ASC_VARIANT(0, 0, 1, 0, 0), ASC_VARIANT(1, 0, 0, 0, 0),
    ASC_VARIANT(0, 1, 0, 0, 0), ASC_VARIANT(0, 0, 0, 0, 0)};
#undef ASC_VARIANT

static void launch_solve(int scheme, int form, int mp, long batch, hipStream_t stream, const ascent_params *dp, const PGeo &g, double *w,
                         int max_iter, double tol) {
  if (scheme == 2) {
    hs_launch_solve(batch, stream, dp, g.K, g.Kp, g.nch, g.term, g.wide, w, max_iter, tol);
    return;
  }
  SolveKernel kernel = g.wide ? p_solve<0, 0, 0, 0, 1> : p_solve<0, 0, 0, 0, 0>;
  for (const SolveVariant &v : solve_variants)
    if (v.scheme == scheme && v.form == form && v.mp == (mp ? 1 : 0) && v.term == g.term && v.wide == g.wide) kernel = v.kernel;
  hipLaunchKernelGGL(kernel, dim3((unsigned)(g.wide ? batch : (batch + NPW - 1) / NPW)), dim3(WAVE), 0, stream, dp, batch, g, w, max_iter, tol);
}

int persist_run_nested(const Call &c, bool wide, const int *levels, int nlev, double *ws, const SolveIO &io, double tol_coarse,
                       double mu_first, double mu_next) {
  const ascent_params *dp = c.dp;
  const long batch = c.batch;
  const int scheme = c.scheme, form = c.form, mp = c.mp, term = c.term;
  hipStream_t stream = c.stream;
  double *region[2] = {ws, (double *)((char *)ws + persist_region1_offset(levels, batch, mp))};
  PGeo g = geo_of(levels[nlev - 1] - 1, form, mp, term, wide, scheme);
  double *w = region[(nlev - 1) & 1];
  hipLaunchKernelGGL(p_init, dim3((unsigned)((g.Kp + WAVE - 1) / WAVE), (unsigned)batch), dim3(WAVE), 0, stream, dp, batch, g, w, io.guess,
                     io.warm, io.mu0, (const double *)nullptr, (const double *)nullptr, 0);
  for (int l = nlev - 1; l >= 0; l--) {
    launch_solve(scheme, form, mp, batch, stream, dp, g, w, io.max_iter, l == 0 ? io.tol : tol_coarse);
    if (l > 0) {
      const PGeo gf = geo_of(levels[l - 1] - 1, form, mp, term, wide, scheme);
      double *wf = region[(l - 1) & 1];
      hipLaunchKernelGGL(p_transfer, dim3((unsigned)((gf.Kp + WAVE - 1) / WAVE), (unsigned)batch), dim3(WAVE), 0, stream, dp, batch, g,
                         (const double *)w, gf, wf, l == nlev - 1 ? mu_first : mu_next);
      g = gf; w = wf;
    }
  }
  hipLaunchKernelGGL(p_finish, dim3((unsigned)((g.K + CH - 1) / CH), (unsigned)((batch + WAVE - 1) / WAVE)), dim3(WAVE, FIN_WAVES), 0, stream, dp, batch, g,
                     (const double *)w, io.traj, io.tf, io.status, io.iters, io.blob);
  ASC_CHK(c.err, c.errlen, hipGetLastError());
  return ASCENT_OK;
}

int persist_probe(const Call &c, bool wide, double *ws, const ProbeIO &io) {
  const PGeo g = geo_of(c.K, c.form, c.mp, c.term, wide, c.scheme);
  const dim3 ng((unsigned)((g.Kp + WAVE - 1) / WAVE), (unsigned)c.batch);
  hipLaunchKernelGGL(p_init, ng, dim3(WAVE), 0, c.stream, c.dp, c.batch, g, ws, io.iterate, 2, 0.1, io.mu, io.dw, 1);
  launch_solve(c.scheme, c.form, c.mp, c.batch, c.stream, c.dp, g, ws, 1000, -1.0);
  hipLaunchKernelGGL(p_probe_out, ng, dim3(WAVE), 0, c.stream, c.batch, g, (const double *)ws, io.step, io.inertia);
  ASC_CHK(c.err, c.errlen, hipGetLastError());
  return ASCENT_OK;
}

int persist_probe_rows(const Call &c, bool wide, double *ws, const ProbeIO &io) {
  const PGeo g = geo_of(c.K, c.form, 0, 0, wide);
  const dim3 ng((unsigned)((g.Kp + WAVE - 1) / WAVE), (unsigned)c.batch);
  hipLaunchKernelGGL(p_init, ng, dim3(WAVE), 0, c.stream, c.dp, c.batch, g, ws, io.iterate, 2, 0.1, io.mu, io.mu, 2);
  launch_solve(c.scheme, c.form, 0, c.batch, c.stream, c.dp, g, ws, 1000, -1.0);
  hipLaunchKernelGGL(p_probe_rows_out, ng, dim3(WAVE), 0, c.stream, c.dp, c.batch, g, (const double *)ws, io.defects, io.jac, io.hess);
  ASC_CHK(c.err, c.errlen, hipGetLastError());
  return ASCENT_OK;
}

}
```

lunar_module_ascent_trajectory_optimiser_amd/csrc/ascent_persist.hpp:

```cpp
#pragma once
#include <hip/hip_runtime.h>
#include <cstddef>
#include "ascent.h"
#include "ascent_host.hpp"

namespace ascent {

size_t persist_ws_bytes(int K, long batch, int mp);

size_t persist_region1_offset(const int *levels, long batch, int mp);
size_t persist_ws_bytes_nested(const int *levels, int nlev, long batch, int mp);
size_t persist_level_bytes_used(int K, long batch, int mp);
int persist_run_nested(const Call &c, bool wide, const int *levels, int nlev, double *ws, const SolveIO &io, double tol_coarse,
                       double mu_first, double mu_next);

int persist_probe(const Call &c, bool wide, double *ws, const ProbeIO &io);

int persist_probe_rows(const Call &c, bool wide, double *ws, const ProbeIO &io);

void hs_launch_solve(long batch, hipStream_t stream, const ascent_params *dp, int K, int Kp, int nch, int term, int wide, double *w, int max_iter, double tol);
int hs_chunk_nodes(int wide);

}
```

lunar_module_ascent_trajectory_optimiser_amd/csrc/ascent_persist_dev.hpp:

```cpp
#pragma once
#include <hip/hip_runtime.h>

#include "ascent.h"
#include "ascent_device.hpp"
#include "ascent_tile.hpp"

namespace {
using namespace ascent;

constexpr int NPW = 4, CH = 16;
constexpr int O_Z = 0, O_U = 7, O_L = 8, O_ZB = 15;
constexpr int O_LU = 21, O_PP = 22, O_PN = 23, O_ZP = 24, O_ZN = 25;
template <int MP>
struct Lay {
  static constexpr int NS = 7 + MP, NIT = 21 + 5 * MP;
  static constexpr int R_IT = 0, R_ST = 2 * NIT, R_KA = 3 * NIT, R_K0 = R_KA + NS, NROWS = R_K0 + 3;
  static constexpr int S_G = 0, S_E = 8, S_H = 12, S_F = 22, S_C = S_F + 7 - MP, S_RZ = S_C + NS, S_GT = S_RZ + NS, S_SC = S_GT + NS;
  static constexpr int S_ROWS = MP ? 56 : 55;
  static constexpr int OUT_ROWS = 11 + MP;
  static_assert(S_SC + (MP ? 3 : 5) <= S_ROWS, "stage rows");
};
constexpr int R_IT = 0;
constexpr int LDW = 65;
enum {
  X_STATE, X_ITERS, X_STATUS, X_CUR, X_FIRST, X_LS, X_MU, X_NUP, X_DW, X_DWL, X_ALPHA, X_ADU, X_PHI0, X_DM, X_C1, X_SL,
  X_RTH, X_DTH, X_DNU3, X_SIG1, X_SIG2, X_RS1, X_RS2, X_CG1, X_CG2,
  X_ITB,
  X_PROBE, X_PDW,
  X_TEVAL,
  X_P,
  X_PEND = X_P + 9,
  X_MV,
  X_S,
  X_D = X_S + 10,
  NSCAL = X_D + 10
};
constexpr int NSCAL_PAD = 64;
static_assert(NSCAL <= NSCAL_PAD, "scalar record");
enum { ST_TRIAL = 0, ST_FACTOR = 1, ST_FACTORED = 2, ST_DONE = 3 };

struct PGeo {
  int K, Kp, nch, form, mp, term, wide;
  __host__ __device__ int nit() const { return mp ? Lay<1>::NIT : Lay<0>::NIT; }
  __host__ __device__ int r_st() const { return 2 * nit(); }
  __host__ __device__ int nrows() const { return mp ? Lay<1>::NROWS : Lay<0>::NROWS; }
  __host__ __device__ size_t nlp_doubles() const { return (size_t)nrows() * Kp + NSCAL_PAD; }
};

template <int SRC>
ASC_DEV double bcast16(double v) {
  const long x = __builtin_amdgcn_mov_dpp(__builtin_bit_cast(long, v), 0x150 + SRC, 0xf, 0xf, false);
  return __builtin_bit_cast(double, x);
}
template <int N>
struct OneHot {
  double m[N];
  ASC_DEV explicit OneHot(int role) {
    ASC_UNROLL
    for (int i = 0; i < N; i++) m[i] = (role == i || (i == 0 && role >= N)) ? 1.0 : 0.0;
  }
  ASC_DEV double pick(const double *v) const {
    double r = m[0] * v[0];
    ASC_UNROLL
    for (int i = 1; i < N; i++) r += m[i] * v[i];
    return r;
  }
};
ASC_DEV void wsync() {
  __builtin_amdgcn_fence(__ATOMIC_RELEASE, "wavefront");
  __builtin_amdgcn_wave_barrier();
  __builtin_amdgcn_fence(__ATOMIC_ACQUIRE, "wavefront");
}
ASC_DEV double gsum16(double v) { v += __shfl_xor(v, 1); v += __shfl_xor(v, 2); v += __shfl_xor(v, 4); v += __shfl_xor(v, 8); return v; }
ASC_DEV double gmax16(double v) { v = fmax(v, __shfl_xor(v, 1)); v = fmax(v, __shfl_xor(v, 2)); v = fmax(v, __shfl_xor(v, 4)); return fmax(v, __shfl_xor(v, 8)); }
ASC_DEV double gmin16(double v) { v = fmin(v, __shfl_xor(v, 1)); v = fmin(v, __shfl_xor(v, 2)); v = fmin(v, __shfl_xor(v, 4)); return fmin(v, __shfl_xor(v, 8)); }
template <int WIDE> ASC_DEV double gsumW(double v) { v = gsum16(v); if constexpr (WIDE) { v += __shfl_xor(v, 16); v += __shfl_xor(v, 32); } return v; }
template <int WIDE> ASC_DEV double gmaxW(double v) { v = gmax16(v); if constexpr (WIDE) { v = fmax(v, __shfl_xor(v, 16)); v = fmax(v, __shfl_xor(v, 32)); } return v; }
template <int WIDE> ASC_DEV double gminW(double v) { v = gmin16(v); if constexpr (WIDE) { v = fmin(v, __shfl_xor(v, 16)); v = fmin(v, __shfl_xor(v, 32)); } return v; }

template <typename PT>
ASC_DEV Scal lds_scal(PT sc, int r0) {
  Scal s;
  s.th = sc[r0 + S_TH]; s.zlt = sc[r0 + S_ZLT]; s.zut = sc[r0 + S_ZUT]; s.s1 = sc[r0 + S_S1]; s.s2 = sc[r0 + S_S2];
  s.zs1 = sc[r0 + S_ZS1]; s.zs2 = sc[r0 + S_ZS2]; s.nu3 = sc[r0 + S_NU3]; s.nu1 = sc[r0 + S_NU1]; s.nu2 = sc[r0 + S_NU2];
  return s;
}
ASC_DEV void put_scal(double *sc, int r0, const Scal &s) {
  sc[r0 + S_TH] = s.th; sc[r0 + S_ZLT] = s.zlt; sc[r0 + S_ZUT] = s.zut; sc[r0 + S_S1] = s.s1; sc[r0 + S_S2] = s.s2;
  sc[r0 + S_ZS1] = s.zs1; sc[r0 + S_ZS2] = s.zs2; sc[r0 + S_NU3] = s.nu3; sc[r0 + S_NU1] = s.nu1; sc[r0 + S_NU2] = s.nu2;
}
ASC_DEV Scal trial_scal(const Der &d, const Scal &s, const Scal &ds, double alpha, double adu, double mu, bool first) {
  Scal t = s;
  if (first) return t;
  t.th += alpha * ds.th; t.s1 += alpha * ds.s1; t.s2 += alpha * ds.s2;
  t.nu3 += alpha * ds.nu3; t.nu1 += alpha * ds.nu1; t.nu2 += alpha * ds.nu2;
  t.zlt = clipz(s.zlt + adu * ds.zlt, t.th - d.tlb, mu);
  t.zut = clipz(s.zut + adu * ds.zut, d.tub - t.th, mu);
  t.zs1 = clipz(s.zs1 + adu * ds.zs1, t.s1, mu);
  t.zs2 = clipz(s.zs2 + adu * ds.zs2, t.s2, mu);
  return t;
}

struct NodeIn {
  double z[7], zp[7], l[7], ln[7], zb[6], u;
  double up, lu, lun, pp, pn, zpp, zpn;
};
template <int MP = 0>
ASC_DEV void load_node(const double *it, int Kp, int K, int k, NodeIn &n, double uinit = 0.0) {
  ASC_UNROLL
  for (int i = 0; i < 7; i++) {
    n.z[i] = it[(O_Z + i) * Kp + k];
    n.l[i] = it[(O_L + i) * Kp + k];
    n.zp[i] = k > 0 ? it[(O_Z + i) * Kp + k - 1] : 0.0;
    n.ln[i] = k + 1 < K ? it[(O_L + i) * Kp + k + 1] : 0.0;
  }
  n.u = it[O_U * Kp + k];
  ASC_UNROLL
  for (int b = 0; b < 6; b++) n.zb[b] = it[(O_ZB + b) * Kp + k];
  if constexpr (MP) {
    n.up = k > 0 ? it[O_U * Kp + k - 1] : uinit;
    n.lu = it[O_LU * Kp + k];
    n.lun = k + 1 < K ? it[O_LU * Kp + k + 1] : 0.0;
    n.pp = it[O_PP * Kp + k]; n.pn = it[O_PN * Kp + k]; n.zpp = it[O_ZP * Kp + k]; n.zpn = it[O_ZN * Kp + k];
  }
}

struct Part {
  double rd, cinf, pmin, pmax, l1, zsum, rth, c1, sl, mv;
  ASC_DEV void clear() { rd = 0.0; cinf = 0.0; pmin = 1e300; pmax = -1e300; l1 = 0.0; zsum = 0.0; rth = 0.0; c1 = 0.0; sl = 0.0; mv = 0.0; }
  template <int MP = 0>
  ASC_DEV void reduce16() {
    rd = gmax16(rd); cinf = gmax16(cinf); pmin = gmin16(pmin); pmax = gmax16(pmax);
    l1 = gsum16(l1); zsum = gsum16(zsum); rth = gsum16(rth); c1 = gsum16(c1); sl = gsum16(sl);
    if constexpr (MP) mv = gsum16(mv);
  }
  template <int MP, int WIDE>
  ASC_DEV void reduceW() {
    rd = gmaxW<WIDE>(rd); cinf = gmaxW<WIDE>(cinf); pmin = gminW<WIDE>(pmin); pmax = gmaxW<WIDE>(pmax);
    l1 = gsumW<WIDE>(l1); zsum = gsumW<WIDE>(zsum); rth = gsumW<WIDE>(rth); c1 = gsumW<WIDE>(c1); sl = gsumW<WIDE>(sl);
    if constexpr (MP) mv = gsumW<WIDE>(mv);
  }
};
struct TrialCtx {
  double alpha, adu, mlo, mhi, dt, be, hT, dcw;
  bool first;
  Scal stt;
};

#ifdef PERSIST_PROFILE
#define PROF_DECL long long prof_[10] = {0, 0, 0, 0, 0, 0, 0, 0, 0, 0}; long long pt_ = clock64();
#define PROF(i_) do { const long long t1_ = clock64(); prof_[i_] += t1_ - pt_; pt_ = t1_; } while (0)
#define PROF_END do { if (blockIdx.x == 0 && threadIdx.x == 0) printf("[persist profile] cycles: A %lld | B eval %lld serial %lld flush %lld | F eval %lld serial %lld post %lld | Adj eval %lld serial %lld | rest %lld\n", prof_[0], prof_[1], prof_[2], prof_[3], prof_[4], prof_[5], prof_[6], prof_[7], prof_[8], prof_[9]); } while (0)
#else
#define PROF_DECL
#define PROF(i_) do { } while (0)
#define PROF_END do { } while (0)
#endif

}
```

lunar_module_ascent_trajectory_optimiser_amd/csrc/ascent_solver.hip:

```cpp
#include <hip/hip_runtime.h>

#include <cstdio>
#include <cstdlib>
#include <cstring>
#include <mutex>
#include <vector>
#include <cmath>

#include "ascent.h"
#include "ascent_host.hpp"
#include "ascent_device.hpp"
#include "ascent_tile.hpp"
#include "ascent_pipeline.hpp"
#include "ascent_dense.hpp"
#include "ascent_blocktri.hpp"
#include "ascent_persist.hpp"
#include "ascent_fused.hpp"
#include "ascent_sens.hpp"
#include "ascent_flight.hpp"
#include "ascent_trim.hpp"
#include "ascent_disperse.hpp"
#include "ascent_guide.hpp"

using namespace ascent;
// ... 830 lines not shown
  int rc = b.flight_like(substeps);
  if (rc) return rc;
  if (!trim_blob_out || !summary_out) { snprintf(g_err, sizeof g_err, "null trim_blob_out or summary_out"); return ASCENT_E_ARG; }
  if (rounds < 0 || rounds > 32) { snprintf(g_err, sizeof g_err, "rounds out of range (1 .. 32, 0 = 6)"); return ASCENT_E_ARG; }
  if ((rc = b.open(device_id, trim_ws_bytes(o->n_nodes - 1, (long)batch)))) return rc;
  if (rounds == 0) rounds = 6;
  if (!(tol > 0.0)) tol = 1e-10;
  double *dout = b.st.out(trim_blob_out, (21 * (size_t)b.K + NSC) * batch), *ds = b.st.out(summary_out, (size_t)ASCENT_TRIM_ROWS * batch);
  if ((rc = b.st.failed()) || (rc = trim_run(b.c, o->terminal, substeps, rounds, tol, b.blob, dout, ds, b.ws))) return rc;
  return b.close();
}

int ascent_disperse_batch(const ascent_params *p, int64_t batch, const ascent_opts *o, const double *sol_blob, int32_t substeps,
                          int32_t samples, const double *xi, const double *sigma, const double *sigma_u, double *stats_out,
                          double *samples_out, int device_id, void *stream_, int ptr_is_device) {
  DisperseIO io{};
  io.blob = sol_blob; io.xi = xi; io.sigma = sigma; io.sigma_u = sigma_u;
  io.stats = stats_out; io.samples_out = samples_out;
  return disperse_call(p, batch, o, substeps, samples, DISPERSE_OPEN, io, device_id, stream_, ptr_is_device);
}

int ascent_guidance_gains(const ascent_params *p, int64_t batch, const ascent_opts *o, const double *sol_blob, int32_t substeps,
                          const double *weights, double *gain_u_out, double *gain_t_out, double *summary_out, double *jac_cl_out,
                          double *jac_u_cl_out, int device_id, void *stream_, int ptr_is_device) {
  GainsIO io{};
  io.blob = sol_blob; io.weights = weights;
  io.gain_u = gain_u_out; io.gain_t = gain_t_out; io.summary = summary_out; io.jac = jac_cl_out; io.jac_u = jac_u_cl_out;
  return gains_call(p, batch, o, substeps, false, io, device_id, stream_, ptr_is_device);
}

int ascent_disperse_guided_batch(const ascent_params *p, int64_t batch, const ascent_opts *o, const double *sol_blob, int32_t substeps,
                                 int32_t samples, const double *xi, const double *sigma, const double *sigma_u, const double *gain_u,
                                 const double *gain_t, const double *stretch_max, double *stats_out, double *samples_out,
                                 int device_id, void *stream_, int ptr_is_device) {
  DisperseIO io{};
  io.blob = sol_blob; io.xi = xi; io.sigma = sigma; io.sigma_u = sigma_u;
  io.gain_u = gain_u; io.gain_t = gain_t; io.stretch_max = stretch_max;
  io.stats = stats_out; io.samples_out = samples_out;
  return disperse_call(p, batch, o, substeps, samples, DISPERSE_GUIDED, io, device_id, stream_, ptr_is_device);
}

int ascent_guidance_feedforward(const ascent_params *p, int64_t batch, const ascent_opts *o, const double *sol_blob, int32_t substeps,
                                const double *weights, const double *ff_dir, const double *ff_know, double *gain_u_out,
                                double *gain_t_out, double *ff_u_out, double *ff_t_out, double *summary_out, double *jac_cl_out,
                                double *jac_u_cl_out, double *jac_nav_out, int device_id, void *stream_, int ptr_is_device) {
  GainsIO io{};
  io.blob = sol_blob; io.weights = weights; io.ff_dir = ff_dir; io.ff_know = ff_know;
  io.gain_u = gain_u_out; io.gain_t = gain_t_out; io.ff_u = ff_u_out; io.ff_t = ff_t_out; io.summary = summary_out;
  io.jac = jac_cl_out; io.jac_u = jac_u_cl_out; io.jac_nav = jac_nav_out;
  return gains_call(p, batch, o, substeps, true, io, device_id, stream_, ptr_is_device);
}

int ascent_disperse_navigated_batch(const ascent_params *p, int64_t batch, const ascent_opts *o, const double *sol_blob, int32_t substeps,
                                    int32_t samples, const double *xi, const double *sigma, const double *sigma_u, const double *gain_u,
                                    const double *gain_t, const double *stretch_max, const double *ff_u, const double *ff_t,
                                    const double *ff_know, const double *xi_nav, const double *sigma_nav, double *stats_out,
                                    double *samples_out, int device_id, void *stream_, int ptr_is_device) {
  DisperseIO io{};
  io.blob = sol_blob; io.xi = xi; io.sigma = sigma; io.sigma_u = sigma_u;
  io.gain_u = gain_u; io.gain_t = gain_t; io.stretch_max = stretch_max;
  io.ff_u = ff_u; io.ff_t = ff_t; io.ff_know = ff_know; io.xi_nav = xi_nav; io.sigma_nav = sigma_nav;
  io.stats = stats_out; io.samples_out = samples_out;
  return disperse_call(p, batch, o, substeps, samples, DISPERSE_NAVIGATED, io, device_id, stream_, ptr_is_device);
}

int ascent_disperse_history_batch(const ascent_params *p, int64_t batch, const ascent_opts *o, const double *sol_blob, int32_t substeps,
                                  int32_t samples, const double *xi, const double *sigma, const double *sigma_u, const double *gain_u,
                                  const double *gain_t, const double *stretch_max, const double *ff_u, const double *ff_t,
                                  const double *ff_know, const double *xi_nav, const double *sigma_nav, int32_t node_stride,
                                  double *stats_out, double *samples_out, double *hist_out, double *hist_samples_out, int device_id,
                                  void *stream_, int ptr_is_device) {
  DisperseIO io{};
  io.blob = sol_blob; io.xi = xi; io.sigma = sigma; io.sigma_u = sigma_u;
  io.gain_u = gain_u; io.gain_t = gain_t; io.stretch_max = stretch_max;
  io.ff_u = ff_u; io.ff_t = ff_t; io.ff_know = ff_know; io.xi_nav = xi_nav; io.sigma_nav = sigma_nav;
  io.stats = stats_out; io.samples_out = samples_out;
  io.node_stride = node_stride; io.hist = hist_out; io.hist_samples = hist_samples_out;
  return disperse_call(p, batch, o, substeps, samples, gain_u ? DISPERSE_NAVIGATED : DISPERSE_OPEN, io, device_id, stream_, ptr_is_device, true);
}

int ascent_kkt_step(const ascent_params *p, int64_t batch, const ascent_opts *o, const double *iterate,
                    const double *mu, const double *delta_w, double *step, int32_t *inertia_out, int device_id) {
  return ascent_kkt_step_path(p, batch, o, iterate, mu, delta_w, step, inertia_out, device_id, ASCENT_PATH_AUTO);
}

int ascent_kkt_solve(int64_t batch, int32_t n, int32_t bs, int32_t nb, const double *diag, const double *lower,
                     const double *upper, const double *border, const double *border_diag, const double *rhs,
                     double *sol, int device_id, int algo) {
  if (batch <= 0 || n < 1 || n > 65535 || bs < 1 || bs > 16 || nb < 0 || nb > 15 || (algo != 0 && algo != 1)) {
    snprintf(g_err, sizeof g_err, "ascent_kkt_solve: need batch > 0, 1 <= n_nodes <= 65535, 1 <= bs <= 16, 0 <= nb <= 15, algo 0 | 1");
    return ASCENT_E_ARG;
  }
  if (!diag || !lower || !upper || !rhs || !sol || (nb && (!border || !border_diag))) { snprintf(g_err, sizeof g_err, "null pointer"); return ASCENT_E_ARG; }
  int rc = check_device(device_id);
  if (rc) return rc;
  std::lock_guard<std::mutex> lock(g_mu[device_id]);
  HIPCHK(hipSetDevice(device_id));
  if ((rc = claim_slot0(device_id))) return rc;
  if ((rc = ensure_ws(g_ws_slot0(device_id), blocktri_ws_bytes(n, (long)batch, algo)))) return rc;
  DeviceWs &w = g_ws_slot0(device_id);
  const size_t nblk = (size_t)batch * n * bs * bs, nbor = (size_t)batch * n * bs * (nb ? nb : 1), nrow = (size_t)n * bs + nb;
  const size_t ny = (size_t)batch * n * bs * (1 + nb);
  std::vector<double> Y(ny);
  Staging st(nullptr, 0);
  const double *dd = st.in(diag, nblk), *dl = st.in(lower, nblk), *du = st.in(upper, nblk);
  const double *db = nb ? st.in(border, nbor) : st.scratch<double>(nbor);
  const double *dr = st.in(rhs, batch * nrow);
  double *dy = st.out(Y.data(), ny);
  if ((rc = st.failed())) return rc;
  int singular = 0;
  rc = blocktri_run((long)batch, n, bs, nb, dd, dl, du, db, dr, w.ws, dy, algo, &singular, 0, w.ev0, w.ev1, g_err, sizeof g_err);
  if (rc) return rc;
  w.launched = true;
  if (singular) { snprintf(g_err, sizeof g_err, "ascent_kkt_solve: singular pivot inside a block (no pivoting)"); return ASCENT_E_ARG; }
  if ((rc = st.finish())) return rc;
  const int nc = 1 + nb;
  std::vector<double> S((size_t)nb * nb), t(nb), yv(nb);
  for (int64_t q = 0; q < batch; q++) {
    const double *Yq = Y.data() + (size_t)q * n * bs * nc;
    const double *Bq = nb ? border + (size_t)q * n * bs * nb : nullptr;
    const double *rq = rhs + (size_t)q * nrow;
    double *xq = sol + (size_t)q * nrow;
    for (int a = 0; a < nb; a++) {
      t[a] = rq[(size_t)n * bs + a];
      for (int b = 0; b < nb; b++) S[(size_t)a * nb + b] = border_diag[((size_t)q * nb + a) * nb + b];
      for (size_t r = 0; r < (size_t)n * bs; r++) {
        const double ba = Bq[r * nb + a];
        t[a] -= ba * Yq[r * nc];
        for (int b = 0; b < nb; b++) S[(size_t)a * nb + b] -= ba * Yq[r * nc + 1 + b];
      }
    }
    for (int a = 0; a < nb; a++) {
      int pv = a;
      for (int r = a + 1; r < nb; r++) if (std::fabs(S[(size_t)r * nb + a]) > std::fabs(S[(size_t)pv * nb + a])) pv = r;
      if (S[(size_t)pv * nb + a] == 0.0) { snprintf(g_err, sizeof g_err, "ascent_kkt_solve: singular border Schur complement"); return ASCENT_E_ARG; }
      if (pv != a) { for (int b = 0; b < nb; b++) std::swap(S[(size_t)a * nb + b], S[(size_t)pv * nb + b]); std::swap(t[a], t[pv]); }
      for (int r = a + 1; r < nb; r++) {
        const double f = S[(size_t)r * nb + a] / S[(size_t)a * nb + a];
        for (int b = a; b < nb; b++) S[(size_t)r * nb + b] -= f * S[(size_t)a * nb + b];
        t[r] -= f * t[a];
      }
    }
    for (int a = nb - 1; a >= 0; a--) {
      double v = t[a];
      for (int b = a + 1; b < nb; b++) v -= S[(size_t)a * nb + b] * yv[b];
      yv[a] = v / S[(size_t)a * nb + a];
    }
    for (size_t r = 0; r < (size_t)n * bs; r++) {
      double v = Yq[r * nc];
      for (int b = 0; b < nb; b++) v -= Yq[r * nc + 1 + b] * yv[b];
      xq[r] = v;
    }
    for (int a = 0; a < nb; a++) xq[(size_t)n * bs + a] = yv[a];
  }
  return ASCENT_OK;
}

}
```

lunar_module_ascent_trajectory_optimiser_amd/distributed.py:

```python
from __future__ import annotations

import numpy as np

from .params import pack
from .solver import solve_batch, solve_batch_torch


def shard_indices(n: int, rank: int, world: int) -> np.ndarray:
    return np.arange(rank, n, world)


def _dist():
    import torch.distributed as dist
    return dist if dist.is_available() and dist.is_initialized() else None


def solve_sharded(params, nt: int = 200, tol: float = 1e-9, max_iter: int = 300, device: int | None = None,
                  gather_traj: bool = False, solver=None, **kw):
    import torch
    P = pack(params)
    n = P.shape[0]
    dist = _dist()
    rank, world = (dist.get_rank(), dist.get_world_size()) if dist else (0, 1)
    if device is None:
        device = rank % max(1, torch.cuda.device_count()) if torch.cuda.is_available() else 0
    idx = shard_indices(n, rank, world)
    m = (n + world - 1) // world
    width = 3 + (10 * nt if gather_traj else 0)
    k = len(idx)
    on_device = solver is None and dist is not None and dist.get_backend() == "nccl"
    failure = None
    if on_device:
        dev = torch.device("cuda", device)
        local = torch.zeros((m + 1, width), dtype=torch.float64, device=dev)
        if k:
            try:
                o = solve_batch_torch(torch.from_numpy(np.ascontiguousarray(P[idx])).to(dev), nt, tol=tol, max_iter=max_iter,
                                      want_traj=gather_traj, **kw)
                local[:k, 0], local[:k, 1], local[:k, 2] = o["tf"], o["status"].double(), o["iters"].double()
                if gather_traj:
                    local[:k, 3:] = o["traj"].permute(2, 0, 1).reshape(k, -1)
            except Exception as e:
                failure = e
                local[m, 0] = 1.0
    else:
        local = np.zeros((m + 1, width))
        if k:
            try:
                res = (solver or solve_batch)(P[idx], nt=nt, tol=tol, max_iter=max_iter, device=device,
                                              want_traj=gather_traj, **kw)
                local[:k, 0], local[:k, 1], local[:k, 2] = res.tf, res.status, res.iters
                if gather_traj:
                    local[:k, 3:] = np.moveaxis(res.traj, 2, 0).reshape(k, -1)
            except Exception as e:
                failure = e
                local[m, 0] = 1.0
    if not dist:
        if failure:
            raise failure
        gathered = [local]
    else:
        if on_device:
            t = local
        else:
            t = torch.from_numpy(local)
            if dist.get_backend() == "nccl":
                t = t.to(torch.device("cuda", device))
        bufs = [torch.empty_like(t) for _ in range(world)] if rank == 0 else None
        dist.gather(t, bufs, dst=0)
        if failure:
            raise failure
        if rank != 0:
            return None
        gathered = [b.cpu().numpy() for b in bufs]
        bad = [r for r, g in enumerate(gathered) if g[m, 0] != 0.0]
        if bad:
            raise RuntimeError(f"solve_sharded: the solver failed on rank(s) {bad}")
    out = np.zeros((n, width))
    for r, g in enumerate(gathered):
        ids = shard_indices(n, r, world)
        out[ids] = g[: len(ids)]
    result = dict(tf=out[:, 0], status=out[:, 1].astype(np.int32), iters=out[:, 2].astype(np.int32))
    if gather_traj:
        result["traj"] = np.moveaxis(out[:, 3:].reshape(n, 10, nt), 0, 2)
    return result
```

lunar_module_ascent_trajectory_optimiser_amd/solver.py:

```python
from __future__ import annotations

import ctypes as C
import dataclasses

import numpy as np

from . import _lib
from .params import PARAM_FIELDS, AscentParams, pack

TRAJ_FIELDS = ("x", "y", "xdot", "ydot", "xdoubledot", "ydoubledot", "angle", "angledot",
               "angledoubledot", "mass")
STATUS_NAMES = {0: "converged", 1: "max_iter", 2: "linesearch_failed", 3: "regularisation_failed"}


def blob_rows(nt: int) -> int:
    return 21 * (nt - 1) + 10


SCHEMES = {"backward_euler": 0, "trapezoid": 1, "hermite_simpson": 2}
TERMINALS = {"reference": 0, "ellipse": 1, "ellipse_free": 2}


FORMULATIONS = {"current": 0, "v1": 1}


def _opts(nt, max_iter, tol, warm_start, mu_init, scheme=0, formulation=0, coarse_nodes=0, terminal=0, path="auto", move_penalty=False):
    scheme = SCHEMES.get(scheme, scheme)
    formulation = FORMULATIONS.get(formulation, formulation)
    terminal = TERMINALS.get(terminal, terminal)
    if path not in ("auto", "dense"):
        raise ValueError('solver path must be "auto" or "dense"')
    return _lib.AscentOptsC(n_nodes=nt, scheme=int(scheme), max_iter=max_iter, warm_start=warm_start, tol=tol,
                            mu_init=mu_init, formulation=int(formulation), coarse_nodes=int(coarse_nodes),
                            terminal=int(terminal), solver_path=_lib.PATHS[path], move_penalty=int(bool(move_penalty)), reserved=0)


def _ptr(a):
    return None if a is None else a.ctypes.data_as(C.c_void_p)


def _blob_call(params, sol_blob, nt, scheme=0, formulation=0, terminal=0, move_penalty=False, what="sol_blob"):
    P = pack(params)
    B = P.shape[0]
    blob = np.ascontiguousarray(sol_blob, dtype=np.float64)
    if blob.shape != (blob_rows(nt), B):
        raise ValueError(f"sol_blob must have shape {(blob_rows(nt), B)}" if what == "sol_blob" else f"{what} has the wrong shape")
    o = _opts(nt, 0, 1.0, 0, 0.0, scheme, formulation, terminal=terminal, move_penalty=move_penalty)
    return _lib.load(), P, B, nt - 1, blob, o


FLIGHT_ROWS = ("miss_position", "miss_velocity", "flown_periapsis_alt", "flown_apoapsis_alt", "nlp_periapsis_alt",
               "nlp_apoapsis_alt", "max_local_position_error", "max_local_velocity_error", "max_local_step", "substeps")


@dataclasses.dataclass
class FlightResult:
    traj: np.ndarray | None
    local_error: np.ndarray | None
    summary: np.ndarray


for _i, _n in enumerate(FLIGHT_ROWS):
    setattr(FlightResult, _n, property(lambda self, _i=_i: self.summary[:, _i]))


JACOBIAN_ROWS = ("x", "y", "xdot", "ydot", "angle", "angledot", "mass", "periapsis_alt", "apoapsis_alt")
TRIM_ROWS = ("status", "rounds", "residual", "residual_before", "delta_tf_seconds", "max_delta_u", "free_controls",
             "flown_periapsis_alt", "flown_apoapsis_alt", "angle_violation")
TRIM_STATUS_NAMES = {0: "converged", 1: "rounds_exhausted", 2: "frozen"}


@dataclasses.dataclass
class FlightJacobian:
    dz0: np.ndarray
    dparams: np.ndarray
    dtf: np.ndarray
    dcontrols: np.ndarray | None

    def predict(self, dparams=None, dtf=None, dcontrols=None, dz0=None) -> np.ndarray:
        out = np.zeros(self.dtf.shape)
        if dparams is not None:
            out += np.einsum("bqc,bc->bq", self.dparams, np.broadcast_to(np.asarray(dparams, dtype=np.float64), self.dparams[:, 0].shape))
        if dtf is not None:
            out += self.dtf * np.broadcast_to(np.asarray(dtf, dtype=np.float64), self.dtf.shape[:1])[:, None]
        if dcontrols is not None:
            if self.dcontrols is None:
                raise ValueError("this FlightJacobian was computed without the control columns")
            out += np.einsum("bqk,bk->bq", self.dcontrols, np.broadcast_to(np.asarray(dcontrols, dtype=np.float64), self.dcontrols[:, 0].shape))
        if dz0 is not None:
            out += np.einsum("bqc,bc->bq", self.dz0, np.broadcast_to(np.asarray(dz0, dtype=np.float64), self.dz0[:, 0].shape))
        return out

    def sigma(self, param_sigma=None, control_sigma=None) -> np.ndarray:
        var = np.zeros(self.dtf.shape)
        if param_sigma is not None:
# ... 475 lines not shown

def eval_nodes(params, iterate: np.ndarray, nt: int = 200, device: int = 0, path="auto", scheme=0, formulation=0):
    L, P, B, K, it, o = _blob_call(params, iterate, nt, scheme, formulation, what="iterate")
    d, j, h = np.empty((7 * K, B)), np.empty((8 * K, B)), np.empty((10 * K, B))
    _lib.check(L.ascent_eval_nodes_path(_ptr(P), B, C.byref(o), _ptr(it), _ptr(d), _ptr(j), _ptr(h), device,
                                        _lib.PATHS[path]))
    return d, j, h


def kkt_step(params, iterate: np.ndarray, mu, delta_w, nt: int = 200, device: int = 0, path="auto", scheme=0,
             formulation=0, terminal=0, move_penalty: bool = False):
    L, P, B, K, it, o = _blob_call(params, iterate, nt, scheme, formulation, terminal, move_penalty, what="iterate")
    mu = np.ascontiguousarray(np.broadcast_to(np.asarray(mu, dtype=np.float64), (B,)))
    dw = np.ascontiguousarray(np.broadcast_to(np.asarray(delta_w, dtype=np.float64), (B,)))
    step = np.empty_like(it)
    inertia = np.empty(B, dtype=np.int32)
    _lib.check(L.ascent_kkt_step_path(_ptr(P), B, C.byref(o), _ptr(it), _ptr(mu), _ptr(dw), _ptr(step), _ptr(inertia),
                                      device, _lib.PATHS[path]))
    return step, inertia


def dense_records(params, iterate: np.ndarray, nt: int = 200, scheme=2, device: int = 0) -> np.ndarray:
    L, P, B, K, it, o = _blob_call(params, iterate, nt, scheme, what="iterate")
    rec = np.empty((B, K, 6, 8, 8))
    _lib.check(L.ascent_dense_records(_ptr(P), B, C.byref(o), _ptr(it), _ptr(rec), device))
    return rec


def coast_batch(params, final_state: np.ndarray, coast_nodes: int = 200, device: int = 0) -> dict:
    L = _lib.load()
    P = pack(params)
    B = P.shape[0]
    fs = np.ascontiguousarray(final_state, dtype=np.float64)
    if fs.shape != (4, B):
        raise ValueError(f"final_state must have shape {(4, B)}")
    traj = np.empty((4, coast_nodes + 1, B)); tf = np.empty(B); aps = np.empty((2, B))
    _lib.check(L.ascent_coast_batch(_ptr(P), B, _ptr(fs), coast_nodes, _ptr(traj), _ptr(tf), _ptr(aps), device, None, 0))
    return dict(traj=traj, tf=tf, periapsis_alt=aps[0], apoapsis_alt=aps[1])


def kkt_solve(diag, lower, upper, rhs, border=None, border_diag=None, algo="pcr", device: int = 0):
    L = _lib.load()
    D = np.ascontiguousarray(diag, dtype=np.float64)
    B, n, bs, _ = D.shape
    Lo = np.ascontiguousarray(lower, dtype=np.float64); Up = np.ascontiguousarray(upper, dtype=np.float64)
    nb = 0 if border is None else int(np.shape(border)[-1])
    r = np.ascontiguousarray(rhs, dtype=np.float64)
    if Lo.shape != D.shape or Up.shape != D.shape or r.shape != (B, n * bs + nb):
        raise ValueError("inconsistent shapes")
    bo = bd = None
    if nb:
        bo = np.ascontiguousarray(border, dtype=np.float64); bd = np.ascontiguousarray(border_diag, dtype=np.float64)
        if bo.shape != (B, n, bs, nb) or bd.shape != (B, nb, nb):
            raise ValueError("inconsistent border shapes")
    sol = np.empty_like(r)
    _lib.check(L.ascent_kkt_solve(B, n, bs, nb, _ptr(D), _ptr(Lo), _ptr(Up), _ptr(bo), _ptr(bd), _ptr(r), _ptr(sol), device,
                                  {"thomas": 0, "pcr": 1}[algo]))
    return sol, L.ascent_last_kernel_ms(device)


def solve_batch_torch(params_t, nt: int = 200, tol: float = 1e-9, max_iter: int = 300, guess_t=None,
                      warm_start: int = 0, mu_init: float = 0.0, want_traj: bool = True, want_blob: bool = False,
                      out: dict | None = None, sync: bool = False, coarse_nodes: int = 0, scheme=0,
                      formulation=0, move_penalty: bool = False, terminal=0, path: str = "auto",
                      sensitivity: bool = False, flight: bool = False) -> dict:
    import torch
    L = _lib.load()
    _lib.require_single_hip_runtime()
    if not (params_t.is_cuda and params_t.dtype == torch.float64 and params_t.is_contiguous()):
        raise ValueError("params_t must be a contiguous float64 CUDA tensor")
    B = params_t.shape[0]
    dev = params_t.device
    rows = blob_rows(nt)
    out = out if out is not None else {}
    def buf(name, shape, dtype):
        t = out.get(name)
        if t is None:
            t = out[name] = torch.empty(shape, dtype=dtype, device=dev)
        elif not (t.device == dev and t.dtype == dtype and tuple(t.shape) == tuple(shape) and t.is_contiguous()):
            raise ValueError(f"out[{name!r}] must be a contiguous {dtype} tensor of shape {tuple(shape)} on {dev}")
        return t
    if params_t.dim() != 2 or params_t.shape[1] != 16:
        raise ValueError("params_t must have shape (batch, 16)")
    if move_penalty and not bool((params_t[:, 15] > 0).all()):
        raise ValueError("move_penalty needs dcost > 0 (column 15 of params_t) for every problem")
    if warm_start not in (0, 1, 2) or (warm_start and guess_t is None):
        raise ValueError("warm_start 1/2 needs guess_t")
    if guess_t is not None and not (guess_t.device == dev and guess_t.dtype == torch.float64 and guess_t.is_contiguous()
                                    and tuple(guess_t.shape) == (rows, B)):
        raise ValueError(f"guess_t must be a contiguous float64 tensor of shape {(rows, B)} on {dev}")
    tf = buf("tf", (B,), torch.float64)
    status = buf("status", (B,), torch.int32)
    iters = buf("iters", (B,), torch.int32)
    traj = buf("traj", (10, nt, B), torch.float64) if want_traj else None
    blob = buf("blob", (rows, B), torch.float64) if want_blob else None
    if (sensitivity or flight) and blob is None:
        blob = torch.empty((rows, B), dtype=torch.float64, device=dev)
    sens = buf("sensitivity", (B, 16), torch.float64) if sensitivity else None
    if flight:
        fsum, ftraj = buf("flight_summary", (B, len(FLIGHT_ROWS)), torch.float64), buf("flight_traj", (B, 10, nt), torch.float64)
        floc = buf("flight_local", (B, nt - 1, 7), torch.float64)
    o = _opts(nt, max_iter, tol, warm_start, mu_init, scheme, formulation, coarse_nodes, terminal, path, move_penalty)
    stream = torch.cuda.current_stream(dev).cuda_stream
    _lib.check(L.ascent_solve_batch(params_t.data_ptr(), B, C.byref(o),
                                    guess_t.data_ptr() if guess_t is not None else None,
                                    traj.data_ptr() if traj is not None else None, tf.data_ptr(), status.data_ptr(),
                                    iters.data_ptr(), blob.data_ptr() if blob is not None else None,
                                    dev.index or 0, C.c_void_p(stream), 1))
    if sensitivity:
        g = torch.empty((16, B), dtype=torch.float64, device=dev)
        _lib.check(L.ascent_param_sensitivity(params_t.data_ptr(), B, C.byref(o), blob.data_ptr(), g.data_ptr(),
                                              dev.index or 0, C.c_void_p(stream), 1))
        J = _penalised_objective(params_t, blob, nt - 1, formulation) if move_penalty else blob[21 * (nt - 1)]
        s_ = g.t() * params_t[:, 11:12]
        s_[:, 11] += J
        sens.copy_(torch.where((status == 0)[:, None], s_, torch.full_like(s_, float("nan"))))
    if flight:
        K = nt - 1
        rs = torch.empty((len(FLIGHT_ROWS), B), dtype=torch.float64, device=dev)
        rt = torch.empty((10, nt, B), dtype=torch.float64, device=dev)
        rl = torch.empty((K, 7, B), dtype=torch.float64, device=dev)
        _lib.check(L.ascent_fly_batch(params_t.data_ptr(), B, C.byref(o), blob.data_ptr(), 0, rt.data_ptr(), rl.data_ptr(),
                                      rs.data_ptr(), dev.index or 0, C.c_void_p(stream), 1))
        ok, nan = status == 0, torch.full((), float("nan"), dtype=torch.float64, device=dev)
        fsum.copy_(torch.where(ok[:, None], rs.t(), nan))
        ftraj.copy_(torch.where(ok[:, None, None], rt.permute(2, 0, 1), nan))
        floc.copy_(torch.where(ok[:, None, None], rl.permute(2, 0, 1), nan))
    if sync:
        torch.cuda.synchronize(dev)
    return out


class _FinalTime:
    fn = None

    @classmethod
    def get(cls):
        if cls.fn is None:
            import torch

            class FinalTime(torch.autograd.Function):
                @staticmethod
                def forward(ctx, params_t, kw):
                    out = solve_batch_torch(params_t.detach().contiguous(), sensitivity=True, want_traj=False,
                                            want_blob=kw.get("move_penalty", False), **kw)
                    T = params_t[:, 11].detach()
                    if kw.get("move_penalty", False):
                        y = T * _penalised_objective(params_t.detach(), out["blob"], kw.get("nt", 200) - 1, kw.get("formulation", 0))
                    else:
                        y = T * out["tf"]
                    y = torch.where(out["status"] == 0, y, torch.full_like(y, float("nan")))
                    ctx.save_for_backward(out["sensitivity"])
                    return y

                @staticmethod
                def backward(ctx, grad_out):
                    (sens,) = ctx.saved_tensors
                    return grad_out[:, None] * sens, None

            cls.fn = FinalTime
        return cls.fn


def final_time(params_t, **solve_kw):
    return _FinalTime.get().apply(params_t, dict(solve_kw))


def default_path(batch: int, nt: int = 200, scheme=0, formulation=0, move_penalty: bool = False, terminal=0) -> str:
# ... 8 lines not shown
```

Measured before the change: 698,800 NLPs/s.

## Use DPP for 16-lane reductions and scans; move dcost validation onto device

```diff
diff --git a/include/ascent.h b/include/ascent.h
--- a/include/ascent.h
+++ b/include/ascent.h
@@ -53,7 +53,8 @@
   ASCENT_CONVERGED = 0,
   ASCENT_MAX_ITER = 1,
   ASCENT_LINESEARCH_FAILED = 2,
-  ASCENT_REGULARISATION_FAILED = 3
+  ASCENT_REGULARISATION_FAILED = 3,
+  ASCENT_INVALID_PROBLEM = 4
 };
 
 #define ASCENT_BLOB_ROWS(n_nodes) (21 * ((n_nodes) - 1) + 10)
@@ -166,6 +167,9 @@
                      const double *upper, const double *border, const double *border_diag, const double *rhs,
                      double *sol, int device_id, int algo);
 
+#define ASCENT_REDUCE_PROBE_ROWS 14
+int ascent_reduce_probe(const double *in, int64_t n, double *out, int device_id);
+
 double ascent_last_kernel_ms(int device_id);
 
 #ifdef __cplusplus
diff --git a/lunar_module_ascent_trajectory_optimiser_amd/_lib.py b/lunar_module_ascent_trajectory_optimiser_amd/_lib.py
--- a/lunar_module_ascent_trajectory_optimiser_amd/_lib.py
+++ b/lunar_module_ascent_trajectory_optimiser_amd/_lib.py
@@ -28,7 +28,9 @@
            "ascent_dense_records", "ascent_coast_batch", "ascent_kkt_solve", "ascent_last_kernel_ms", "ascent_default_path",
            "ascent_workspace_layout", "ascent_param_sensitivity", "ascent_fly_batch", "ascent_flight_jacobian",
            "ascent_trim_batch", "ascent_disperse_batch", "ascent_guidance_gains", "ascent_disperse_guided_batch",
-           "ascent_guidance_feedforward", "ascent_disperse_navigated_batch", "ascent_disperse_history_batch")
+           "ascent_guidance_feedforward", "ascent_disperse_navigated_batch", "ascent_disperse_history_batch",
+           "ascent_reduce_probe")
+REDUCE_PROBE_ROWS = 14
 PATHS = {"auto": 0, "fused": 1, "split_lane": 2, "split_wide": 3, "dense": 4, "persist": 5}
 
 _lib = None
@@ -119,6 +121,8 @@
     L.ascent_dense_records.argtypes = [C.c_void_p, C.c_int64, C.POINTER(AscentOptsC), C.c_void_p, C.c_void_p, C.c_int]
     L.ascent_kkt_solve.restype = C.c_int
     L.ascent_kkt_solve.argtypes = [C.c_int64, C.c_int32, C.c_int32, C.c_int32] + [C.c_void_p] * 7 + [C.c_int, C.c_int]
+    L.ascent_reduce_probe.restype = C.c_int
+    L.ascent_reduce_probe.argtypes = [C.c_void_p, C.c_int64, C.c_void_p, C.c_int]
     L.ascent_coast_batch.restype = C.c_int
     L.ascent_coast_batch.argtypes = [C.c_void_p, C.c_int64, C.c_void_p, C.c_int32, C.c_void_p, C.c_void_p, C.c_void_p,
                                      C.c_int, C.c_void_p, C.c_int]
diff --git a/lunar_module_ascent_trajectory_optimiser_amd/csrc/ascent_dense.hip b/lunar_module_ascent_trajectory_optimiser_amd/csrc/ascent_dense.hip
--- a/lunar_module_ascent_trajectory_optimiser_amd/csrc/ascent_dense.hip
+++ b/lunar_module_ascent_trajectory_optimiser_amd/csrc/ascent_dense.hip
@@ -114,7 +114,7 @@
   if (g.dc) {
     double up = (k > 0 && warm) ? guess[(7L * K + k - 1) * batch + p] : 0.0;
     if (k > 0 && !probe) up = push_in(up, -1.0, 1.0);
-    const double dl = u - up, eps = warm ? 1e-4 : 1e-2, dc = params[p].dcost;
+    const double dl = u - up, eps = warm ? 1e-4 : 1e-2, dc = params[p].dcost > 0.0 ? params[p].dcost : 1.0;
     it[O_LU * K + k] = 0.0;
     it[O_PP * K + k] = fmax(dl, 0.0) + eps; it[O_PN * K + k] = fmax(-dl, 0.0) + eps;
     it[O_ZP * K + k] = dc; it[O_ZN * K + k] = dc;
@@ -147,6 +147,7 @@
   sc[X_STATE] = ST_TRIAL; sc[X_FIRST] = 1.0; sc[X_STATUS] = ASCENT_MAX_ITER;
   sc[X_MU] = probe ? probe_mu[p] : ((asked_warm && !warm) ? 0.1 : mu_init);
   sc[X_NUP] = 1.0;
+  if (g.dc && !(params[p].dcost > 0.0)) { sc[X_STATE] = ST_DONE; sc[X_STATUS] = ASCENT_INVALID_PROBLEM; }
 }
 
 struct QMap { int q; double c; };
diff --git a/lunar_module_ascent_trajectory_optimiser_amd/csrc/ascent_hs.hip b/lunar_module_ascent_trajectory_optimiser_amd/csrc/ascent_hs.hip
--- a/lunar_module_ascent_trajectory_optimiser_amd/csrc/ascent_hs.hip
+++ b/lunar_module_ascent_trajectory_optimiser_amd/csrc/ascent_hs.hip
@@ -412,12 +412,7 @@
     for (int i = 0; i < 7; i++) rc[i] = cc[i] + Jth[i] * dth;
     x0m = -rc[IM];
   }
-  double incl = x0m;
-  ASC_UNROLL
-  for (int sft = 1; sft < (WIDE ? 64 : 16); sft *= 2) {
-    const double t = __shfl_up(incl, sft, WIDE ? 64 : 16);
-    if (nl >= sft) incl += t;
-  }
+  const double incl = scanW<WIDE>(x0m, nl);
   const double dzm_k = carry_m + incl, dzm_p = dzm_k - x0m;
   carry_m += WIDE ? __shfl(incl, HCW - 1) : bcast16<HCH - 1>(incl);
   if (on) {
diff --git a/lunar_module_ascent_trajectory_optimiser_amd/csrc/ascent_persist.hip b/lunar_module_ascent_trajectory_optimiser_amd/csrc/ascent_persist.hip
--- a/lunar_module_ascent_trajectory_optimiser_amd/csrc/ascent_persist.hip
+++ b/lunar_module_ascent_trajectory_optimiser_amd/csrc/ascent_persist.hip
@@ -16,6 +16,7 @@
 namespace {
 
 
+ASC_DEV bool bad_weight(const ascent_params &prm) { return !(prm.dcost > 0.0); }
 ASC_DEV void start_move(double *w, int Kp, int k, double u, double up, bool warm, double dcw) {
   const double dl = u - up, eps = warm ? 1e-4 : 1e-2;
   w[(R_IT + O_LU) * Kp + k] = 0.0;
@@ -108,7 +109,7 @@
     const double ha = 0.5 * d.aub, f0 = (double)kk / K * 0.5;
     double up = kk == 0 ? (g.form == 1 ? -1.0 : 0.0) : warm ? guess[(7L * K + kk - 1) * batch + p] : (g.form == 1 ? f0 / ha - 1.0 : 0.0);
     if (kk > 0 && !probe) up = push_in(up, -1.0, 1.0);
-    start_move(w, Kp, k, u, up, warm != 0, g.form == 1 ? params[p].dcost * ha : params[p].dcost);
+    start_move(w, Kp, k, u, up, warm != 0, bad_weight(params[p]) ? 1.0 : g.form == 1 ? params[p].dcost * ha : params[p].dcost);
   }
   if (k != K - 1) return;
   double *sc = w + (size_t)g.nrows() * Kp;
@@ -125,6 +126,7 @@
   sc[X_STATE] = ST_TRIAL; sc[X_FIRST] = 1.0; sc[X_STATUS] = ASCENT_MAX_ITER;
   sc[X_MU] = (asked_warm && !warm) ? 0.1 : mu_init; sc[X_NUP] = 1.0;
   if (probe) { sc[X_MU] = probe_mu[p]; sc[X_PDW] = probe_dw[p]; sc[X_PROBE] = (double)probe_kind; }
+  if (g.mp && bad_weight(params[p])) { sc[X_STATE] = ST_DONE; sc[X_STATUS] = ASCENT_INVALID_PROBLEM; }
 }
 
 __global__ __launch_bounds__(WAVE) void p_transfer(const ascent_params *params, long batch, PGeo gc, const double *wsc, PGeo gf,
@@ -136,6 +138,7 @@
   double *wf = wsf + (size_t)p * gf.nlp_doubles();
   const Der d = derive_t(params[p], gf.term);
   const int warm = (int)scc[X_STATUS] == ASCENT_CONVERGED ? 2 : 0;
+  const bool invalid = (int)scc[X_STATUS] == ASCENT_INVALID_PROBLEM;
   const double *ic = wc + (size_t)((int)scc[X_CUR] * gc.nit()) * Kpc;
   double z[7], l[7], zb[6], u = 0.0, up = 0.0;
   const int kk = k < Kf ? k : Kf - 1;
@@ -174,7 +177,7 @@
   if (gf.mp) {
     if (kk == 0) up = gf.form == 1 ? -1.0 : 0.0;
     else if (!warm && gf.form == 1) up = push_in((double)kk / Kf * 0.5 / (0.5 * d.aub) - 1.0, -1.0, 1.0);
-    start_move(wf, Kpf, k, u, up, warm != 0, gf.form == 1 ? params[p].dcost * 0.5 * d.aub : params[p].dcost);
+    start_move(wf, Kpf, k, u, up, warm != 0, invalid ? 1.0 : gf.form == 1 ? params[p].dcost * 0.5 * d.aub : params[p].dcost);
   }
   if (k != Kf - 1) return;
   double *sc = wf + (size_t)gf.nrows() * Kpf;
@@ -186,6 +189,7 @@
   sc[X_STATE] = ST_TRIAL; sc[X_FIRST] = 1.0; sc[X_STATUS] = ASCENT_MAX_ITER;
   sc[X_MU] = warm ? mu : 0.1; sc[X_NUP] = 1.0;
   sc[X_ITB] = scc[X_ITB] + scc[X_ITERS];
+  if (invalid) { sc[X_STATE] = ST_DONE; sc[X_STATUS] = ASCENT_INVALID_PROBLEM; }
 }
 
 constexpr int FIN_WAVES = 8, FIN_SUB = CH / FIN_WAVES;
@@ -240,6 +244,22 @@
       for (int f = 0; f < 10; f++) traj[((long)f * nt + k + 1) * batch + p] = v[f];
     }
   }
+}
+
+__global__ __launch_bounds__(WAVE) void p_reduce_probe(const double *in, long n, double *out) {
+  const long r = blockIdx.x;
+  if (r >= n) return;
+  const int lane = threadIdx.x;
+  const double v = in[r * WAVE + lane];
+  double *o = out + r * ASCENT_REDUCE_PROBE_ROWS * WAVE + lane;
+  const double s16 = gsum16_shfl(v), x16 = gmax16_shfl(v), n16 = gmin16_shfl(v);
+  o[0 * WAVE] = gsum16(v); o[1 * WAVE] = gmax16(v); o[2 * WAVE] = gmin16(v);
+  o[3 * WAVE] = s16; o[4 * WAVE] = x16; o[5 * WAVE] = n16;
+  o[6 * WAVE] = gsumW<1>(v); o[7 * WAVE] = gmaxW<1>(v); o[8 * WAVE] = gminW<1>(v);
+  { double t = s16; t += __shfl_xor(t, 16); t += __shfl_xor(t, 32); o[9 * WAVE] = t; }
+  { double t = x16; t = fmax(t, __shfl_xor(t, 16)); t = fmax(t, __shfl_xor(t, 32)); o[10 * WAVE] = t; }
+  { double t = n16; t = fmin(t, __shfl_xor(t, 16)); t = fmin(t, __shfl_xor(t, 32)); o[11 * WAVE] = t; }
+  o[12 * WAVE] = scan16(v, lane & 15); o[13 * WAVE] = scan_shfl<16>(v, lane & 15);
 }
 
 __global__ __launch_bounds__(WAVE) void p_probe_out(long batch, PGeo g, const double *ws, double *step, int *inertia) {
@@ -503,7 +523,7 @@
               trial_node<SCHEME, FORM, MP, TERM>(d, K, Kp, k, n, dn, t, live, in, P);
             }
           }
-          P.template reduceW<MP, WIDE>();
+          P.template reduceW<MP, WIDE, MP>();
         }
         double rd = P.rd, cinf = P.cinf, pmin = P.pmin, pmax = P.pmax, l1 = P.l1, zsum = P.zsum;
         const double rth = 1.0 + P.rth, c1 = P.c1, sl = P.sl;
@@ -848,8 +868,8 @@
         PROF(3);
       }
       const double U0 = bcast16<RL>(U), U1 = bcast16<RL + 1>(U), V1 = bcast16<RL + 1>(V), U2 = bcast16<RL + 2>(U), V2 = bcast16<RL + 2>(V);
-      k10 = gsumW<WIDE>(k10); k11 = gsumW<WIDE>(k11); k12 = gsumW<WIDE>(k12); k20 = gsumW<WIDE>(k20); k22 = gsumW<WIDE>(k22);
-      bad = (int)gmaxW<WIDE>((double)bad);
+      k10 = gsumW<WIDE, MP>(k10); k11 = gsumW<WIDE, MP>(k11); k12 = gsumW<WIDE, MP>(k12); k20 = gsumW<WIDE, MP>(k20); k22 = gsumW<WIDE, MP>(k22);
+      bad = (int)gmaxW<WIDE, MP>((double)bad);
       if (probe_rows) {
         if (act && role == 0) sc[X_STATE] = ST_DONE;
       } else if (act) {
@@ -946,12 +966,7 @@
             }
             if constexpr (MP) du00 -= ka[7] * x0u;
           }
-          double incl = x0[IM];
-          ASC_UNROLL
-          for (int sft = 1; sft < CHN; sft *= 2) {
-            const double t = __shfl_up(incl, sft, CHN);
-            if (nl >= sft) incl += t;
-          }
+          const double incl = scanW<WIDE, MP>(x0[IM], nl);
           const double dzm_k = carry_m + incl, dzm_p = dzm_k - x0[IM];
           carry_m += WIDE ? __shfl(incl, 63) : bcast16<15>(incl);
           if (on) {
@@ -1103,10 +1118,10 @@
           wsync();
           PROF(6);
         }
-        rmax = gmaxW<WIDE>(rmax); gsum = gsumW<WIDE>(gsum); adu = gminW<WIDE>(adu);
-        if constexpr (MP) { gmove = gsumW<WIDE>(gmove); clu = gsumW<WIDE>(clu); }
+        rmax = gmaxW<WIDE, MP>(rmax); gsum = gsumW<WIDE, MP>(gsum); adu = gminW<WIDE, MP>(adu);
+        if constexpr (MP) { gmove = gsumW<WIDE, MP>(gmove); clu = gsumW<WIDE, MP>(clu); }
         ASC_UNROLL
-        for (int i = 0; i < 7; i++) dzK[i] = gsumW<WIDE>(dzK[i]);
+        for (int i = 0; i < 7; i++) dzK[i] = gsumW<WIDE, MP>(dzK[i]);
         double zK[7];
         ASC_UNROLL
         for (int i = 0; i < 7; i++) zK[i] = it[(O_Z + i) * Kp + K - 1];
@@ -1293,8 +1308,8 @@
           }
           PROF(0);
         }
-        P.template reduceW<MP, WIDE>();
-        ccl = gsumW<WIDE>(ccl);
+        P.template reduceW<MP, WIDE, MP>();
+        ccl = gsumW<WIDE, MP>(ccl);
         if (act) {
           cl += ccl;
           const Terminal &tm = tmK;
@@ -1437,4 +1452,10 @@
   return ASCENT_OK;
 }
 
-}
+int reduce_probe_run(const double *in, long n, double *out, hipStream_t stream, char *err, size_t errlen) {
+  hipLaunchKernelGGL(p_reduce_probe, dim3((unsigned)n), dim3(WAVE), 0, stream, in, n, out);
+  ASC_CHK(err, errlen, hipGetLastError());
+  return ASCENT_OK;
+}
+
+}
diff --git a/lunar_module_ascent_trajectory_optimiser_amd/csrc/ascent_persist.hpp b/lunar_module_ascent_trajectory_optimiser_amd/csrc/ascent_persist.hpp
--- a/lunar_module_ascent_trajectory_optimiser_amd/csrc/ascent_persist.hpp
+++ b/lunar_module_ascent_trajectory_optimiser_amd/csrc/ascent_persist.hpp
@@ -18,6 +18,8 @@
 
 int persist_probe_rows(const Call &c, bool wide, double *ws, const ProbeIO &io);
 
+int reduce_probe_run(const double *in, long n, double *out, hipStream_t stream, char *err, size_t errlen);
+
 void hs_launch_solve(long batch, hipStream_t stream, const ascent_params *dp, int K, int Kp, int nch, int term, int wide, double *w, int max_iter, double tol);
 int hs_chunk_nodes(int wide);
 
diff --git a/lunar_module_ascent_trajectory_optimiser_amd/csrc/ascent_persist_dev.hpp b/lunar_module_ascent_trajectory_optimiser_amd/csrc/ascent_persist_dev.hpp
--- a/lunar_module_ascent_trajectory_optimiser_amd/csrc/ascent_persist_dev.hpp
+++ b/lunar_module_ascent_trajectory_optimiser_amd/csrc/ascent_persist_dev.hpp
@@ -71,12 +71,47 @@
   __builtin_amdgcn_wave_barrier();
   __builtin_amdgcn_fence(__ATOMIC_ACQUIRE, "wavefront");
 }
-ASC_DEV double gsum16(double v) { v += __shfl_xor(v, 1); v += __shfl_xor(v, 2); v += __shfl_xor(v, 4); v += __shfl_xor(v, 8); return v; }
-ASC_DEV double gmax16(double v) { v = fmax(v, __shfl_xor(v, 1)); v = fmax(v, __shfl_xor(v, 2)); v = fmax(v, __shfl_xor(v, 4)); return fmax(v, __shfl_xor(v, 8)); }
-ASC_DEV double gmin16(double v) { v = fmin(v, __shfl_xor(v, 1)); v = fmin(v, __shfl_xor(v, 2)); v = fmin(v, __shfl_xor(v, 4)); return fmin(v, __shfl_xor(v, 8)); }
-template <int WIDE> ASC_DEV double gsumW(double v) { v = gsum16(v); if constexpr (WIDE) { v += __shfl_xor(v, 16); v += __shfl_xor(v, 32); } return v; }
-template <int WIDE> ASC_DEV double gmaxW(double v) { v = gmax16(v); if constexpr (WIDE) { v = fmax(v, __shfl_xor(v, 16)); v = fmax(v, __shfl_xor(v, 32)); } return v; }
-template <int WIDE> ASC_DEV double gminW(double v) { v = gmin16(v); if constexpr (WIDE) { v = fmin(v, __shfl_xor(v, 16)); v = fmin(v, __shfl_xor(v, 32)); } return v; }
+ASC_DEV double gsum16_shfl(double v) { v += __shfl_xor(v, 1); v += __shfl_xor(v, 2); v += __shfl_xor(v, 4); v += __shfl_xor(v, 8); return v; }
+ASC_DEV double gmax16_shfl(double v) { v = fmax(v, __shfl_xor(v, 1)); v = fmax(v, __shfl_xor(v, 2)); v = fmax(v, __shfl_xor(v, 4)); return fmax(v, __shfl_xor(v, 8)); }
+ASC_DEV double gmin16_shfl(double v) { v = fmin(v, __shfl_xor(v, 1)); v = fmin(v, __shfl_xor(v, 2)); v = fmin(v, __shfl_xor(v, 4)); return fmin(v, __shfl_xor(v, 8)); }
+constexpr int DPP_XOR1 = 0xB1, DPP_XOR2 = 0x4E, DPP_ROW_SHR = 0x110, DPP_ROW_MIRROR = 0x140, DPP_HALF_MIRROR = 0x141;
+template <int CTRL>
+ASC_DEV double dpp16(double v) {
+  const long x = __builtin_amdgcn_mov_dpp(__builtin_bit_cast(long, v), CTRL, 0xf, 0xf, false);
+  return __builtin_bit_cast(double, x);
+}
+ASC_DEV double gsum16(double v) { v += dpp16<DPP_XOR1>(v); v += dpp16<DPP_XOR2>(v); v += dpp16<DPP_HALF_MIRROR>(v); v += dpp16<DPP_ROW_MIRROR>(v); return v; }
+ASC_DEV double gmax16(double v) { v = fmax(v, dpp16<DPP_XOR1>(v)); v = fmax(v, dpp16<DPP_XOR2>(v)); v = fmax(v, dpp16<DPP_HALF_MIRROR>(v)); return fmax(v, dpp16<DPP_ROW_MIRROR>(v)); }
+ASC_DEV double gmin16(double v) { v = fmin(v, dpp16<DPP_XOR1>(v)); v = fmin(v, dpp16<DPP_XOR2>(v)); v = fmin(v, dpp16<DPP_HALF_MIRROR>(v)); return fmin(v, dpp16<DPP_ROW_MIRROR>(v)); }
+template <int SFT>
+ASC_DEV double shr16(double v) {
+  const long x = __builtin_bit_cast(long, v);
+  const int lo = (int)x, hi = (int)(x >> 32);
+  const unsigned rlo = (unsigned)__builtin_amdgcn_update_dpp(lo, lo, DPP_ROW_SHR + SFT, 0xf, 0xf, false);
+  const unsigned rhi = (unsigned)__builtin_amdgcn_update_dpp(hi, hi, DPP_ROW_SHR + SFT, 0xf, 0xf, false);
+  return __builtin_bit_cast(double, (long)(((unsigned long)rhi << 32) | rlo));
+}
+ASC_DEV double scan16(double v, int nl) {
+  double t;
+  t = shr16<1>(v); if (nl >= 1) v += t;
+  t = shr16<2>(v); if (nl >= 2) v += t;
+  t = shr16<4>(v); if (nl >= 4) v += t;
+  t = shr16<8>(v); if (nl >= 8) v += t;
+  return v;
+}
+template <int W>
+ASC_DEV double scan_shfl(double v, int nl) {
+  ASC_UNROLL
+  for (int sft = 1; sft < W; sft *= 2) {
+    const double t = __shfl_up(v, sft, W);
+    if (nl >= sft) v += t;
+  }
+  return v;
+}
+template <int WIDE, int DPP = 1> ASC_DEV double scanW(double v, int nl) { if constexpr (WIDE) return scan_shfl<64>(v, nl); else if constexpr (DPP) return scan16(v, nl); else return scan_shfl<16>(v, nl); }
+template <int WIDE, int DPP = 1> ASC_DEV double gsumW(double v) { v = DPP ? gsum16(v) : gsum16_shfl(v); if constexpr (WIDE) { v += __shfl_xor(v, 16); v += __shfl_xor(v, 32); } return v; }
+template <int WIDE, int DPP = 1> ASC_DEV double gmaxW(double v) { v = DPP ? gmax16(v) : gmax16_shfl(v); if constexpr (WIDE) { v = fmax(v, __shfl_xor(v, 16)); v = fmax(v, __shfl_xor(v, 32)); } return v; }
+template <int WIDE, int DPP = 1> ASC_DEV double gminW(double v) { v = DPP ? gmin16(v) : gmin16_shfl(v); if constexpr (WIDE) { v = fmin(v, __shfl_xor(v, 16)); v = fmin(v, __shfl_xor(v, 32)); } return v; }
 
 template <typename PT>
 ASC_DEV Scal lds_scal(PT sc, int r0) {
@@ -134,11 +169,11 @@
     l1 = gsum16(l1); zsum = gsum16(zsum); rth = gsum16(rth); c1 = gsum16(c1); sl = gsum16(sl);
     if constexpr (MP) mv = gsum16(mv);
   }
-  template <int MP, int WIDE>
+  template <int MP, int WIDE, int DPP = 1>
   ASC_DEV void reduceW() {
-    rd = gmaxW<WIDE>(rd); cinf = gmaxW<WIDE>(cinf); pmin = gminW<WIDE>(pmin); pmax = gmaxW<WIDE>(pmax);
-    l1 = gsumW<WIDE>(l1); zsum = gsumW<WIDE>(zsum); rth = gsumW<WIDE>(rth); c1 = gsumW<WIDE>(c1); sl = gsumW<WIDE>(sl);
-    if constexpr (MP) mv = gsumW<WIDE>(mv);
+    rd = gmaxW<WIDE, DPP>(rd); cinf = gmaxW<WIDE, DPP>(cinf); pmin = gminW<WIDE, DPP>(pmin); pmax = gmaxW<WIDE, DPP>(pmax);
+    l1 = gsumW<WIDE, DPP>(l1); zsum = gsumW<WIDE, DPP>(zsum); rth = gsumW<WIDE, DPP>(rth); c1 = gsumW<WIDE, DPP>(c1); sl = gsumW<WIDE, DPP>(sl);
+    if constexpr (MP) mv = gsumW<WIDE, DPP>(mv);
   }
 };
 struct TrialCtx {
diff --git a/lunar_module_ascent_trajectory_optimiser_amd/csrc/ascent_solver.hip b/lunar_module_ascent_trajectory_optimiser_amd/csrc/ascent_solver.hip
--- a/lunar_module_ascent_trajectory_optimiser_amd/csrc/ascent_solver.hip
+++ b/lunar_module_ascent_trajectory_optimiser_amd/csrc/ascent_solver.hip
@@ -936,6 +936,20 @@
 int ascent_kkt_step(const ascent_params *p, int64_t batch, const ascent_opts *o, const double *iterate,
                     const double *mu, const double *delta_w, double *step, int32_t *inertia_out, int device_id) {
   return ascent_kkt_step_path(p, batch, o, iterate, mu, delta_w, step, inertia_out, device_id, ASCENT_PATH_AUTO);
+}
+
+int ascent_reduce_probe(const double *in, int64_t n, double *out, int device_id) {
+  if (!in || !out || n <= 0 || n > 65535) { snprintf(g_err, sizeof g_err, "ascent_reduce_probe: null pointer or n outside 1 .. 65535"); return ASCENT_E_ARG; }
+  int rc = check_device(device_id);
+  if (rc) return rc;
+  std::lock_guard<std::mutex> lock(g_mu[device_id]);
+  HIPCHK(hipSetDevice(device_id));
+  Staging st(nullptr, 0);
+  const double *din = st.in(in, (size_t)n * WAVE);
+  double *dout = st.out(out, (size_t)n * ASCENT_REDUCE_PROBE_ROWS * WAVE);
+  if ((rc = st.failed())) return rc;
+  if ((rc = reduce_probe_run(din, (long)n, dout, nullptr, g_err, sizeof g_err))) return rc;
+  return st.finish();
 }
 
 int ascent_kkt_solve(int64_t batch, int32_t n, int32_t bs, int32_t nb, const double *diag, const double *lower,
diff --git a/lunar_module_ascent_trajectory_optimiser_amd/distributed.py b/lunar_module_ascent_trajectory_optimiser_amd/distributed.py
--- a/lunar_module_ascent_trajectory_optimiser_amd/distributed.py
+++ b/lunar_module_ascent_trajectory_optimiser_amd/distributed.py
@@ -35,6 +35,8 @@
         local = torch.zeros((m + 1, width), dtype=torch.float64, device=dev)
         if k:
             try:
+                if kw.get("move_penalty") and not np.all(P[idx][:, 15] > 0):
+                    raise ValueError("move_penalty needs dcost > 0 (column 15 of the parameter sets) for every problem")
                 o = solve_batch_torch(torch.from_numpy(np.ascontiguousarray(P[idx])).to(dev), nt, tol=tol, max_iter=max_iter,
                                       want_traj=gather_traj, **kw)
                 local[:k, 0], local[:k, 1], local[:k, 2] = o["tf"], o["status"].double(), o["iters"].double()
diff --git a/lunar_module_ascent_trajectory_optimiser_amd/solver.py b/lunar_module_ascent_trajectory_optimiser_amd/solver.py
--- a/lunar_module_ascent_trajectory_optimiser_amd/solver.py
+++ b/lunar_module_ascent_trajectory_optimiser_amd/solver.py
@@ -10,7 +10,7 @@
 
 TRAJ_FIELDS = ("x", "y", "xdot", "ydot", "xdoubledot", "ydoubledot", "angle", "angledot",
                "angledoubledot", "mass")
-STATUS_NAMES = {0: "converged", 1: "max_iter", 2: "linesearch_failed", 3: "regularisation_failed"}
+STATUS_NAMES = {0: "converged", 1: "max_iter", 2: "linesearch_failed", 3: "regularisation_failed", 4: "invalid_problem"}
 
 
 def blob_rows(nt: int) -> int:
@@ -652,8 +652,6 @@
         return t
     if params_t.dim() != 2 or params_t.shape[1] != 16:
         raise ValueError("params_t must have shape (batch, 16)")
-    if move_penalty and not bool((params_t[:, 15] > 0).all()):
-        raise ValueError("move_penalty needs dcost > 0 (column 15 of params_t) for every problem")
     if warm_start not in (0, 1, 2) or (warm_start and guess_t is None):
         raise ValueError("warm_start 1/2 needs guess_t")
     if guess_t is not None and not (guess_t.device == dev and guess_t.dtype == torch.float64 and guess_t.is_contiguous()
```

Measured after the change: 713,300 NLPs/s (median of 6 runs). 1.02x the previous value.
